# hmetaxa/MVTopicModel

Hardware: AMD Instinct MI355X
Metric: gibbs_tokens_per_sec (higher is better)
Workload: dtype f64

## Files before the change

### include/mvhdp.h

```cpp
#ifndef MVHDP_H
#define MVHDP_H

#include <stddef.h>
#include <stdint.h>

#ifdef __cplusplus
extern "C" {
#endif

#define MVHDP_MAX_MODALITIES 8
#define MVHDP_MAX_TOPICS     2048
#define MVHDP_UNASSIGNED_TOPIC (-1)

typedef enum {
    MVHDP_OK = 0,
    MVHDP_ERR_INVALID_ARG   = -1,
    MVHDP_ERR_STATE         = -2,
    MVHDP_ERR_HIP           = -3,
    MVHDP_ERR_NO_DEVICE     = -4,
    MVHDP_ERR_NEGATIVE_COUNT= -5,
    MVHDP_ERR_UNSUPPORTED   = -6
} mvhdp_status;

typedef struct mvhdp_ctx* mvhdp_handle;
// ... 95 lines not shown
int mvhdp_build_counts(mvhdp_handle h);
int mvhdp_build_trees(mvhdp_handle h);
int mvhdp_build_inference_trees(mvhdp_handle h);
int mvhdp_init_assignments_from_trees(mvhdp_handle h, uint64_t seed);
int mvhdp_get_counts(mvhdp_handle h, int32_t m, int32_t* n_wk , int32_t* n_k );
int mvhdp_set_counts(mvhdp_handle h, int32_t m, const int32_t* n_wk, const int32_t* n_k);
int mvhdp_get_tree(mvhdp_handle h, int32_t m, int32_t type, double* tree );
int mvhdp_get_doc_topic_hist(mvhdp_handle h, int32_t m, int32_t* hist , int32_t hist_len,
                             int32_t* doc_len_counts , int32_t len_len);

int mvhdp_get_count_histogram(mvhdp_handle h, int32_t m, int32_t* hist, int32_t len);
int mvhdp_view_overlap_sums(mvhdp_handle h, double* sums );
int mvhdp_model_log_likelihood(mvhdp_handle h, double* log_likelihood );
int mvhdp_gamma_doc_statistics(mvhdp_handle h, int32_t m, double gamma_m, uint64_t seed, uint32_t round, double* qs, double* qw);
int mvhdp_dp_table_statistics(mvhdp_handle h, int32_t m, const int32_t* hist , int32_t hist_len, const double* conc ,
                              uint64_t seed, uint32_t round, double* mk , uint8_t* active );
int mvhdp_antoniak_draws(mvhdp_handle h, int32_t n, const int32_t* items , const double* conc , uint64_t seed, uint32_t round, int32_t* tables );
int mvhdp_doc_topic_proportions(mvhdp_handle h, const double* view_weights , int64_t d0, int64_t d1, double* out );

#define MVHDP_DIAG_MAX_TOP_WORDS 64
#define MVHDP_DIAG_PROPORTIONS   7
#define MVHDP_DIAG_TOKENS             0
#define MVHDP_DIAG_DOCUMENT_ENTROPY   1
#define MVHDP_DIAG_WORD_LENGTH        2
#define MVHDP_DIAG_COHERENCE          3
#define MVHDP_DIAG_NORM_DISCR_WEIGHT  4
#define MVHDP_DIAG_DISCR_WEIGHT       5
#define MVHDP_DIAG_UNIFORM_DIST       6
#define MVHDP_DIAG_CORPUS_DIST        7
#define MVHDP_DIAG_EFF_NUM_WORDS      8
#define MVHDP_DIAG_TOKEN_DOC_DIFF     9
#define MVHDP_DIAG_RANK_1_DOCS       10
#define MVHDP_DIAG_ALLOCATION_RATIO  11
#define MVHDP_DIAG_ALLOCATION_COUNT  12
#define MVHDP_DIAG_ROWS              13
typedef struct {
    int32_t num_top_words;
    const int32_t* word_length;
} mvhdp_diag_args;
typedef struct {
    double*  scores;
    double*  word_scores;
    int32_t* codoc;
    int32_t* top_types;
    int32_t* top_counts;
    int32_t* nonzero;
    int32_t* num_rank1_docs;
    int32_t* num_nonzero_docs;
    int32_t* num_docs_at_proportions;
    double*  sum_count_log_count;
    int32_t* word_type_counts;
    int64_t* num_tokens;
    double*  discr_weight_per_view;
} mvhdp_diag_out;
int mvhdp_top_words(mvhdp_handle h, int32_t m, int32_t n, int32_t* types , int32_t* counts , int32_t* nonzero );
int mvhdp_discr_weights(mvhdp_handle h, double* per_view , int32_t m, double* type_weight );
int mvhdp_diagnostics(mvhdp_handle h, const mvhdp_diag_args* args, mvhdp_diag_out* out);

int mvhdp_sweep(mvhdp_handle h, uint32_t sweep_idx, uint64_t seed, uint32_t flags,
                const double* p_override, const mvhdp_debug* dbg, mvhdp_sweep_stats* stats);
int mvhdp_sweep_many(mvhdp_handle h, uint32_t first_idx, int32_t n, uint64_t seed, uint32_t flags, mvhdp_sweep_stats* stats );
int mvhdp_apply_delta(mvhdp_handle h, int32_t activated_topic, int32_t activated_modality);
int mvhdp_apply_delta_begin(mvhdp_handle h);
int mvhdp_apply_delta_rows(mvhdp_handle h, int64_t row_begin, int64_t row_end);
int mvhdp_apply_delta_end(mvhdp_handle h, int32_t activated_topic, int32_t activated_modality);
int mvhdp_get_birth_keys(mvhdp_handle h, int64_t* keys );
int mvhdp_activate_births(mvhdp_handle h, const int64_t* keys );
int mvhdp_trees_current(mvhdp_handle h);
int mvhdp_get_view_weights(mvhdp_handle h, double* p );

typedef struct {
    int32_t force_primary;
    int32_t narrow;
    int32_t walk_fixed;
    int32_t single_stream;
    int32_t live16;
    int32_t single_wave;
    double  walk_theta[MVHDP_MAX_MODALITIES];
    double  primary_min_share;
    int32_t learnt_walk_step[4];
    double  tree_branch_share[MVHDP_MAX_MODALITIES];
    int32_t live_overlap;
    int32_t live_rows;
} mvhdp_tuning;
int mvhdp_get_tuning(mvhdp_handle h, mvhdp_tuning* t);
int mvhdp_set_tuning(mvhdp_handle h, const mvhdp_tuning* t);

typedef struct {
    int32_t num_topics, num_modalities;
    int64_t num_entities;
    int64_t max_entity_tokens;
    int64_t entities_longer_than[5];
    uint64_t tokens_by_list_rounds[17];
    uint64_t entities_by_class[8];
    uint32_t flags;
    int32_t debug, batch, trees_current;
    int32_t num_cus;
    int32_t kernel_registers[6][3];
    int32_t inactive_topics;
} mvhdp_plan_input;
typedef struct {
    int32_t status;
    int32_t segments, primary_class, register_resident, need_full_trees, dominant_class;
    int64_t routed_prefix;
    int32_t class_used[6], class_map[6], class_stream[6], class_grid[6], class_walk[6], class_narrow[6], class_register_resident[6];
    int64_t class_lds_bytes[6];
    double  class_theta0[6];
    int32_t delta16, live_rows;
} mvhdp_plan_output;
int mvhdp_plan_probe(const mvhdp_plan_input* in, const mvhdp_tuning* tuning , mvhdp_plan_output* out);
int mvhdp_tuner_probe(int32_t num_modalities, const double* tree_branch_share , const double* u1_hist ,
                      const double* ns_by_step , int32_t n_sweeps, int32_t group, int32_t* steps_out );

typedef struct mvhdp_group_ctx* mvhdp_group;
#define MVHDP_UNIQUE_ID_BYTES 128
typedef struct {
    int32_t local_members;
    int32_t local_devices;
    int32_t ranks, first_rank;
    int32_t rccl;
    int32_t rccl_version;
    int32_t exchange_chunks;
    int32_t exchange_packed;
    double  last_exchange_ms;
    int64_t last_exchange_bytes;
} mvhdp_group_info;
int mvhdp_group_create(int32_t n, const mvhdp_handle* members, mvhdp_group* out);
int mvhdp_group_unique_id(uint8_t* id );
int mvhdp_group_create_rank(mvhdp_handle member, const uint8_t* id , int32_t rank, int32_t nranks, mvhdp_group* out);
int mvhdp_group_destroy(mvhdp_group g);
const char* mvhdp_group_last_error(mvhdp_group g);
int mvhdp_group_get_info(mvhdp_group g, mvhdp_group_info* info);
int mvhdp_group_set_exchange_chunks(mvhdp_group g, int32_t chunks );
int mvhdp_group_build_counts(mvhdp_group g);
int mvhdp_group_sweep(mvhdp_group g, uint32_t sweep_idx, uint64_t seed, uint32_t flags, mvhdp_sweep_stats* stats);
#define MVHDP_SWEEP_ASYNC_EXCHANGE 0x100u
int mvhdp_group_drain(mvhdp_group g);
int mvhdp_group_abort(mvhdp_group g);

int mvhdp_group_set_hyper(mvhdp_group g, const mvhdp_hyper* hy);
int mvhdp_group_log_likelihood(mvhdp_group g, double* log_likelihood );
int mvhdp_group_doc_topic_hist(mvhdp_group g, int32_t m, int32_t* hist , int32_t hist_len,
                               int32_t* doc_len_counts , int32_t len_len);
int mvhdp_group_count_histogram(mvhdp_group g, int32_t m, int32_t* hist, int32_t len);
int mvhdp_group_view_overlap_sums(mvhdp_group g, double* sums );
int mvhdp_group_gamma_doc_statistics(mvhdp_group g, int32_t m, double gamma_m, uint64_t seed, uint32_t round, double* qs, double* qw);
int mvhdp_group_diagnostics(mvhdp_group g, const mvhdp_diag_args* args, mvhdp_diag_out* out);

int mvhdp_device_buffer(mvhdp_handle h, mvhdp_buffer which, void** dev_ptr, size_t* bytes);
int mvhdp_counts_written(mvhdp_handle h);
int mvhdp_set_stream(mvhdp_handle h, void* hip_stream );
int mvhdp_synchronize(mvhdp_handle h);

#ifdef __cplusplus
}
#endif
#endif
```

### mvtopicmodel_amd/_lib.py

```python
import ctypes as C
import os

_HERE = os.path.dirname(os.path.abspath(__file__))
LIB_PATH = os.path.join(_HERE, "lib", "libmvhdp.so")

MAX_M = 8

ABI_SYMBOLS = [
    "mvhdp_create", "mvhdp_destroy", "mvhdp_last_error", "mvhdp_version",
    "mvhdp_set_corpus", "mvhdp_set_assignments", "mvhdp_set_view_presence", "mvhdp_get_assignments",
    "mvhdp_set_hyper", "mvhdp_get_alpha", "mvhdp_build_counts", "mvhdp_build_trees",
    "mvhdp_build_inference_trees", "mvhdp_init_assignments_from_trees",
    "mvhdp_get_counts", "mvhdp_set_counts", "mvhdp_get_tree", "mvhdp_get_doc_topic_hist",
    "mvhdp_get_count_histogram", "mvhdp_view_overlap_sums", "mvhdp_model_log_likelihood", "mvhdp_doc_topic_proportions",
    "mvhdp_gamma_doc_statistics", "mvhdp_dp_table_statistics", "mvhdp_antoniak_draws",
    "mvhdp_top_words", "mvhdp_discr_weights", "mvhdp_diagnostics",
    "mvhdp_sweep", "mvhdp_sweep_many", "mvhdp_get_tuning", "mvhdp_set_tuning", "mvhdp_plan_probe", "mvhdp_tuner_probe",
    "mvhdp_apply_delta", "mvhdp_apply_delta_begin", "mvhdp_apply_delta_rows", "mvhdp_apply_delta_end",
    "mvhdp_get_birth_keys", "mvhdp_activate_births",
    "mvhdp_trees_current", "mvhdp_get_view_weights",
    "mvhdp_device_buffer", "mvhdp_counts_written", "mvhdp_set_stream", "mvhdp_synchronize",
    "mvhdp_group_create", "mvhdp_group_unique_id", "mvhdp_group_create_rank", "mvhdp_group_destroy", "mvhdp_group_last_error",
    "mvhdp_group_get_info", "mvhdp_group_set_exchange_chunks", "mvhdp_group_build_counts", "mvhdp_group_sweep", "mvhdp_group_abort", "mvhdp_group_drain",
    "mvhdp_group_set_hyper", "mvhdp_group_log_likelihood", "mvhdp_group_doc_topic_hist", "mvhdp_group_count_histogram",
    "mvhdp_group_view_overlap_sums", "mvhdp_group_gamma_doc_statistics", "mvhdp_group_diagnostics",
]

UNIQUE_ID_BYTES = 128


class MvhdpError(RuntimeError):
    def __init__(self, code, msg):
        super().__init__(f"mvhdp error {code}: {msg}")
        self.code = code


class Config(C.Structure):
    _fields_ = [("num_topics", C.c_int32), ("num_modalities", C.c_int32),
                ("num_types", C.c_int32 * MAX_M), ("device", C.c_int32),
                ("doc_id_base", C.c_int64), ("flags", C.c_uint32)]


class HyperC(C.Structure):
    _fields_ = [("alpha", C.c_void_p),
                ("alpha_sum", C.c_double * MAX_M), ("beta", C.c_double * MAX_M),
                ("beta_sum", C.c_double * MAX_M), ("gamma", C.c_double * MAX_M),
                ("p_a", (C.c_double * MAX_M) * MAX_M), ("p_b", (C.c_double * MAX_M) * MAX_M),
                ("inactive", C.c_void_p)]


class SweepStatsC(C.Structure):
    _fields_ = [("tokens", C.c_int64), ("changed", C.c_int64), ("new_mass_cnt", C.c_int64),
                ("topic_doc_mass_cnt", C.c_int64), ("word_ftree_mass_cnt", C.c_int64),
                ("oov_skipped", C.c_int64), ("aborted_docs", C.c_int64), ("exact_fallbacks", C.c_int64),
                ("activated_topic", C.c_int32), ("activated_modality", C.c_int32),
                ("activation_key", C.c_int64), ("sweep_kernel_ms", C.c_double), ("total_ms", C.c_double),
                ("activations", C.c_int32), ("reserved", C.c_int32)]


class DebugC(C.Structure):
    _fields_ = [("tok_dbg", C.c_void_p * MAX_M), ("n_trace", C.c_int32),
                ("trace_doc", C.c_void_p), ("trace_view", C.c_void_p), ("trace_pos", C.c_void_p),
                ("trace_out", C.c_void_p)]


class TuningC(C.Structure):
    _fields_ = [("force_primary", C.c_int32), ("narrow", C.c_int32), ("walk_fixed", C.c_int32), ("single_stream", C.c_int32),
                ("live16", C.c_int32), ("single_wave", C.c_int32),
                ("walk_theta", C.c_double * MAX_M), ("primary_min_share", C.c_double),
                ("learnt_walk_step", C.c_int32 * 4), ("tree_branch_share", C.c_double * MAX_M),
                ("live_overlap", C.c_int32), ("live_rows", C.c_int32)]


class GroupInfoC(C.Structure):
    _fields_ = [("local_members", C.c_int32), ("local_devices", C.c_int32), ("ranks", C.c_int32), ("first_rank", C.c_int32),
                ("rccl", C.c_int32), ("rccl_version", C.c_int32), ("exchange_chunks", C.c_int32), ("exchange_packed", C.c_int32),
                ("last_exchange_ms", C.c_double), ("last_exchange_bytes", C.c_int64)]


class PlanInputC(C.Structure):
    _fields_ = [("num_topics", C.c_int32), ("num_modalities", C.c_int32), ("num_entities", C.c_int64),
                ("max_entity_tokens", C.c_int64), ("entities_longer_than", C.c_int64 * 5),
                ("tokens_by_list_rounds", C.c_uint64 * 17), ("entities_by_class", C.c_uint64 * 8),
                ("flags", C.c_uint32), ("debug", C.c_int32), ("batch", C.c_int32), ("trees_current", C.c_int32),
                ("num_cus", C.c_int32), ("kernel_registers", (C.c_int32 * 3) * 6), ("inactive_topics", C.c_int32)]


class PlanOutputC(C.Structure):
    _fields_ = [("status", C.c_int32), ("segments", C.c_int32), ("primary_class", C.c_int32), ("register_resident", C.c_int32),
                ("need_full_trees", C.c_int32), ("dominant_class", C.c_int32), ("routed_prefix", C.c_int64),
                ("class_used", C.c_int32 * 6), ("class_map", C.c_int32 * 6), ("class_stream", C.c_int32 * 6),
                ("class_grid", C.c_int32 * 6), ("class_walk", C.c_int32 * 6), ("class_narrow", C.c_int32 * 6),
                ("class_register_resident", C.c_int32 * 6), ("class_lds_bytes", C.c_int64 * 6), ("class_theta0", C.c_double * 6),
                ("delta16", C.c_int32), ("live_rows", C.c_int32)]


DIAG_MAX_TOP_WORDS = 64
DIAG_PROPORTIONS = 7
DIAG_ROWS = ["tokens", "document_entropy", "word-length", "coherence", "normDiscrWeight", "discrWeight", "uniform_dist",
             "corpus_dist", "eff_num_words", "token-doc-diff", "rank_1_docs", "allocation_ratio", "allocation_count"]


class DiagArgsC(C.Structure):
    _fields_ = [("num_top_words", C.c_int32), ("word_length", C.c_void_p)]


class DiagOutC(C.Structure):
    _fields_ = [("scores", C.c_void_p), ("word_scores", C.c_void_p), ("codoc", C.c_void_p), ("top_types", C.c_void_p),
                ("top_counts", C.c_void_p), ("nonzero", C.c_void_p), ("num_rank1_docs", C.c_void_p), ("num_nonzero_docs", C.c_void_p),
                ("num_docs_at_proportions", C.c_void_p), ("sum_count_log_count", C.c_void_p), ("word_type_counts", C.c_void_p),
                ("num_tokens", C.c_void_p), ("discr_weight_per_view", C.c_void_p)]


_lib = None
_preloaded = []


def _torch_lib_dir():
    import importlib.util
    try:
        spec = importlib.util.find_spec("torch")
    except (ImportError, ValueError):
        return None
    if spec is None or not spec.submodule_search_locations:
        return None
    d = os.path.join(list(spec.submodule_search_locations)[0], "lib")
    return d if os.path.isdir(d) else None


def mapped_runtime_libraries():
    found = {"libamdhip64": set(), "libhsa-runtime64": set(), "librccl": set()}
    try:
        with open("/proc/self/maps") as f:
            for line in f:
                path = line.rsplit(None, 1)[-1] if "/" in line else ""
                base = os.path.basename(path)
                for name in found:
                    if base.startswith(name + ".so"):
                        found[name].add(os.path.realpath(path))
    except OSError:
        pass
    return {k: sorted(v) for k, v in found.items()}


def _preload_one_hip_runtime():
    d = _torch_lib_dir()
    if d is None:
        return False
    already = mapped_runtime_libraries()
    if already["libamdhip64"] or already["libhsa-runtime64"]:
        return False
    path = os.path.join(d, "libamdhip64.so")
    if not os.path.exists(path):
        return False
# ... 96 lines not shown
```

### mvtopicmodel_amd/csrc/mvhdp_api.hip

```cpp
#include "mvhdp_ctx.h"

static thread_local std::string g_create_error;

static std::mutex g_reg_mutex;
static std::set<mvhdp_ctx*>* g_live = nullptr;
static bool g_exiting = false, g_atexit_registered = false;
static void release_device_resources(mvhdp_ctx* h);

static void mvhdp_at_exit()
{
    std::lock_guard<std::mutex> lk(g_reg_mutex);
    g_exiting = true;
    if (g_live) for (mvhdp_ctx* h : *g_live) release_device_resources(h);
}

static void register_handle(mvhdp_ctx* h)
{
    std::lock_guard<std::mutex> lk(g_reg_mutex);
    if (!g_live) g_live = new std::set<mvhdp_ctx*>();
    g_live->insert(h);
    if (!g_atexit_registered) { atexit(mvhdp_at_exit); g_atexit_registered = true; }
}

bool mvhdp_is_live(mvhdp_ctx* h)
{
    std::lock_guard<std::mutex> lk(g_reg_mutex);
    return g_live && g_live->count(h) != 0;
}

static void read_environment(mvhdp_ctx* h)
{
    if (const char* f = getenv("MVHDP_FORCE_RMAX")) { const int v = atoi(f); if (v == 1 || v == 2 || v == 4 || v == 8 || v == 16 || v == 32) h->tu.force_primary = v; }
    if (const char* f = getenv("MVHDP_NARROW")) h->tu.narrow = atoi(f) != 0 ? -1 : 0;
    if (const char* f = getenv("MVHDP_SINGLE_STREAM")) h->tu.single_stream = atoi(f) != 0;
    if (const char* f = getenv("MVHDP_SIDE_PRIORITY")) h->side_priority = atoi(f);
    if (const char* f = getenv("MVHDP_LIVE16")) h->tu.live16 = atoi(f);
    if (const char* f = getenv("MVHDP_LIVE_OVERLAP")) h->tu.live_overlap = atoi(f);
    if (const char* f = getenv("MVHDP_LIVE_ROWS")) h->tu.live_rows = atoi(f);
    if (const char* f = getenv("MVHDP_LIVE_ROWS_THETA")) h->tu.live_rows_theta = atof(f);
    if (const char* f = getenv("MVHDP_COEF_LDS_KB")) h->tu.coef_lds_max_bytes = std::max(0, std::min(64, atoi(f))) * 1024;
    if (const char* f = getenv("MVHDP_LIVE_ROWS_SEGMENTS")) h->tu.live_rows_segments = std::max(1, std::min(255, atoi(f)));
    if (const char* f = getenv("MVHDP_WIDEST_ON_MAIN")) h->tu.widest_on_main = atoi(f) != 0;
    if (const char* f = getenv("MVHDP_NARROW_WIDE")) h->tu.narrow_wide = atoi(f) != 0;
    if (const char* f = getenv("MVHDP_LIVE_TREE_EVERY")) h->live_tree_every = std::max(1, atoi(f));
    if (const char* f = getenv("MVHDP_GATE_PCT")) { const int v = atoi(f); if (v >= 5 && v <= 95) h->gate_pct = v; }
    if (const char* f = getenv("MVHDP_FOUR_ROUND_ON_C")) h->tu.four_round_on_c = atoi(f);
    if (const char* f = getenv("MVHDP_DELTA16")) h->tu.delta16 = atoi(f) != 0;
    if (const char* f = getenv("MVHDP_FORK_DELAY_US")) h->tu.fork_delay_us = std::max(0, std::min(1000, atoi(f)));
    if (const char* f = getenv("MVHDP_FORCE_MODE")) { if (!strcmp(f, "serial")) h->tu.single_stream = 1; }
    if (const char* f = getenv("MVHDP_PRIMARY_MIN_SHARE")) { const double v = atof(f); if (v > 0.0 && v <= 1.0) h->tu.primary_min_share = v; }
    if (const char* t = getenv("MVHDP_WALK_THETA")) {
        int m = 0;
        for (const char* q = t; *q && m < MVHDP_MAXM; m++) {
            h->tu.walk_theta[m] = atof(q);
            while (*q && *q != ',') q++;
            if (*q == ',') q++;
        }
        for (; m < MVHDP_MAXM; m++) h->tu.walk_theta[m] = 0.0;
        h->tu.walk_fixed = 1;
    }
    h->dbg_env = getenv("MVHDP_DEBUG") != nullptr;
}

extern "C" const char* mvhdp_version(void) { return "mvhdp 0.1 (gfx950)"; }

extern "C" const char* mvhdp_last_error(mvhdp_handle h) { return (h && mvhdp_is_live(h)) ? h->err.c_str() : g_create_error.c_str(); }

extern "C" int mvhdp_create(const mvhdp_config* cfg, mvhdp_handle* out)
{
    if (!cfg || !out) { g_create_error = "null argument"; return MVHDP_ERR_INVALID_ARG; }
    *out = nullptr;
    const int K = cfg->num_topics, M = cfg->num_modalities;
    if (K < 1 || K > MVHDP_MAX_TOPICS || M < 1 || M > MVHDP_MAX_MODALITIES) {
        g_create_error = "num_topics must be in [1,2048] and num_modalities in [1,8]";
        return MVHDP_ERR_INVALID_ARG;
    }
    for (int m = 0; m < M; m++) if (cfg->num_types[m] < 1) { g_create_error = "num_types[m] must be >= 1"; return MVHDP_ERR_INVALID_ARG; }
    for (int m = 0; m < M; m++) if (cfg->num_types[m] >= (1 << 29)) { g_create_error = "num_types[m] must be below 2^29"; return MVHDP_ERR_INVALID_ARG; }
    if (cfg->doc_id_base < 0 || cfg->doc_id_base >= (1LL << 29)) { g_create_error = "doc_id_base out of range"; return MVHDP_ERR_INVALID_ARG; }
    int ndev = 0;
    if (hipGetDeviceCount(&ndev) != hipSuccess || ndev <= 0 || cfg->device < 0 || cfg->device >= ndev) {
        g_create_error = "no usable HIP device (the sweep has no CPU fallback)";
        return MVHDP_ERR_NO_DEVICE;
    }
    hipDeviceProp_t prop;
    if (hipGetDeviceProperties(&prop, cfg->device) != hipSuccess) { g_create_error = "hipGetDeviceProperties failed"; return MVHDP_ERR_HIP; }
    if (strncmp(prop.gcnArchName, "gfx950", 6) != 0) {
        g_create_error = std::string("device is ") + prop.gcnArchName + ", this library is built for gfx950 only";
        return MVHDP_ERR_NO_DEVICE;
    }
    mvhdp_ctx* h = new mvhdp_ctx();
    register_handle(h);
    h->cfg = *cfg;
    h->device = cfg->device;
    h->num_cus = prop.multiProcessorCount;
    h->max_lds = 160 * 1024;
    MvModel& mm = h->mm;
    mm.K = K; mm.M = M;
    mm.rowbase[0] = 0;
    for (int m = 0; m < M; m++) { mm.V[m] = cfg->num_types[m]; mm.rowbase[m + 1] = mm.rowbase[m] + cfg->num_types[m]; }
    mm.doc_id_base = cfg->doc_id_base;
    mm.first_inactive = -1;
    mm.D = -1;
#define CREATE_HIP(call) do { hipError_t e_ = (call); if (e_ != hipSuccess) { \
    g_create_error = std::string(#call) + ": " + hipGetErrorString(e_); mvhdp_destroy(h); return MVHDP_ERR_HIP; } } while (0)
    CREATE_HIP(hipSetDevice(h->device));
    CREATE_HIP(hipStreamCreateWithFlags(&h->stream, hipStreamNonBlocking));
    h->own_stream = true;
    for (auto& e : h->ev) CREATE_HIP(hipEventCreate(&e));
    const int64_t nrows = mm.rowbase[M];
    const size_t cbytes = (size_t)(nrows * K + (int64_t)M * K + MVHDP_TAIL_WORDS) * sizeof(int32_t);
    CREATE_HIP(hipMalloc(&mm.counts, cbytes));
    CREATE_HIP(hipMalloc(&mm.delta, cbytes));
    CREATE_HIP(hipMemset(mm.counts, 0, cbytes));
    CREATE_HIP(hipMalloc(&mm.counts16, (size_t)nrows * K * sizeof(uint16_t) + 64));
    CREATE_HIP(hipMemset(mm.counts16, 0, (size_t)nrows * K * sizeof(uint16_t)));
    CREATE_HIP(hipMalloc(&mm.delta16, (size_t)(nrows * K + 2) * sizeof(uint16_t)));
    CREATE_HIP(hipMemsetD16(mm.delta16, (unsigned short)0x8000, (size_t)(nrows * K + 2)));
    CREATE_HIP(hipMalloc(&mm.heavy, (size_t)nrows));
    CREATE_HIP(hipMemset(mm.heavy, 1, (size_t)nrows));
    CREATE_HIP(hipMemset(mm.delta, 0, cbytes));
    CREATE_HIP(hipMalloc(&mm.trees, (size_t)nrows * 2 * K * sizeof(double)));
    CREATE_HIP(hipMalloc(&mm.root, (size_t)nrows * sizeof(double)));
    CREATE_HIP(hipMalloc(&mm.mass0, (size_t)nrows * sizeof(float)));
    CREATE_HIP(hipMemset(mm.mass0, 0, (size_t)nrows * sizeof(float)));
    CREATE_HIP(hipMalloc(&mm.coef, (size_t)M * (((K + 7) & ~7) + K + 8) * sizeof(float)));
    {
        const int nlev = (K > 1) ? (32 - __builtin_clz((unsigned)(K - 1))) : 0;
        mm.dt_f = nlev ? ((nlev - 1) % 3) + 1 : 0;
        mm.dt_nbd = 1; mm.dt_base[0] = 0; mm.dt_depth[0] = 0;
        int nblk = 1;
        for (int dep = mm.dt_f; nlev && dep < nlev; dep += 3) {
            mm.dt_base[mm.dt_nbd] = nblk; mm.dt_depth[mm.dt_nbd] = dep; mm.dt_nbd++;
            nblk += 1 << dep;
        }
        mm.dt_nblk = nblk;
        CREATE_HIP(hipMalloc(&mm.dtab, (size_t)nrows * nblk * 8 * sizeof(double)));
    }
    CREATE_HIP(hipMalloc(&h->d_alpha, (size_t)M * (K + 1) * sizeof(double)));
    CREATE_HIP(hipMalloc(&h->d_inactive, (size_t)K));
    CREATE_HIP(hipMemset(h->d_inactive, 0, (size_t)K));
    CREATE_HIP(hipMalloc(&h->d_births, (size_t)(2 + 2 * K) * sizeof(int32_t)));
    CREATE_HIP(hipMemset(h->d_births, 0, (size_t)(2 + 2 * K) * sizeof(int32_t)));
    CREATE_HIP(hipMalloc(&h->d_birth_keys, (size_t)K * sizeof(long long)));
    CREATE_HIP(hipMalloc(&h->d_birth_table, (size_t)K * sizeof(long long)));
    {
        const std::vector<long long> none((size_t)K, LLONG_MAX);
        CREATE_HIP(hipMemcpy(h->d_birth_table, none.data(), (size_t)K * sizeof(long long), hipMemcpyHostToDevice));
    }
    CREATE_HIP(hipMalloc(&h->d_ctl, CTL_WORDS * sizeof(unsigned long long)));
    CREATE_HIP(hipMemset(h->d_ctl, 0, CTL_WORDS * sizeof(unsigned long long)));
    h->d_stats = h->d_ctl;
    h->d_act_key = (long long*)(h->d_ctl + ST_COUNT);
    h->d_ovf_meta = (unsigned int*)(h->d_ctl + ST_COUNT + 1);
    h->d_doc_counter = h->d_ctl + ST_COUNT + 1 + META_WORDS64;
    CREATE_HIP(hipHostMalloc((void**)&h->h_ctl, CTL_WORDS * sizeof(unsigned long long), hipHostMallocDefault));
    for (int c = 0; c < MVHDP_N_CLASSES; c++)
        for (int f = 0; f < 3; f++) h->regs.regs[c][f] = mvhdp_sweep_kernel_regs(c, f);
    read_environment(h);
    mm.alpha = h->d_alpha;
    mm.inactive = h->d_inactive;
    h->h_alpha.assign((size_t)M * (K + 1), 0.0);
    h->h_inactive.assign((size_t)K, 0);
    h->wt.init_defaults(K);
    *out = h;
    return MVHDP_OK;
}

static void release_device_resources(mvhdp_ctx* h)
{
    if (h->device_released) return;
    h->device_released = true;
    hipSetDevice(h->device);
    if (h->stream) hipStreamSynchronize(h->stream);
    auto fr = [](auto*& p) { if (p) { hipFree((void*)p); p = nullptr; } };
    for (int m = 0; m < MVHDP_MAXM; m++) { fr(h->d_doc_off[m]); fr(h->d_tok[m]); fr(h->d_z[m]); fr(h->d_carry[m]); fr(h->d_present[m]); }
    fr(h->mm.counts); fr(h->mm.delta16); fr(h->mm.counts16); fr(h->mm.heavy); fr(h->mm.delta); fr(h->mm.trees); fr(h->mm.root); fr(h->mm.coef); fr(h->mm.mass0); fr(h->d_births); fr(h->d_birth_keys); fr(h->d_birth_table); fr(h->mm.dtab); fr(h->mm.p);
    fr(h->d_alpha); fr(h->d_inactive); fr(h->d_ctl);
    if (h->h_ctl) { hipHostFree(h->h_ctl); h->h_ctl = nullptr; }
    h->d_stats = nullptr; h->d_act_key = nullptr; h->d_doc_counter = nullptr; h->d_ovf_meta = nullptr;
    fr(h->d_doc_order); fr(h->d_lists); fr(h->d_nslots); fr(h->d_stats_many); fr(h->d_heavy_list); fr(h->d_heavy_ctl);
    if (h->ev_rf_go) { hipEventDestroy(h->ev_rf_go); h->ev_rf_go = nullptr; }
    if (h->ev_rf_done) { hipEventDestroy(h->ev_rf_done); h->ev_rf_done = nullptr; }
    if (h->rf_stream) { hipStreamDestroy(h->rf_stream); h->rf_stream = nullptr; }
    fr(h->ov.counts2); fr(h->ov.counts16_2); fr(h->ov.dtab2); fr(h->ov.root2); fr(h->ov.trees2); fr(h->ov.delta2); fr(h->ov.delta3); fr(h->ov.ctl2); fr(h->ov.lists2);
    for (auto& e : h->ov.ev_seg) if (e) { hipEventDestroy(e); e = nullptr; }
    if (h->ov.ev_start) { hipEventDestroy(h->ov.ev_start); h->ov.ev_start = nullptr; }
    if (h->ov.x1) { hipStreamDestroy(h->ov.x1); h->ov.x1 = nullptr; }
    if (h->ov.xa) { hipStreamDestroy(h->ov.xa); h->ov.xa = nullptr; }
    for (auto& e : h->ev_many) if (e) { hipEventDestroy(e); e = nullptr; }
    for (auto& e : h->ev) if (e) { hipEventDestroy(e); e = nullptr; }
    if (h->ev_fork) { hipEventDestroy(h->ev_fork); h->ev_fork = nullptr; }
    for (auto& e : h->ev_join) if (e) { hipEventDestroy(e); e = nullptr; }
    for (auto& st : h->side) if (st) { hipStreamDestroy(st); st = nullptr; }
    if (h->own_stream && h->stream) hipStreamDestroy(h->stream);
    h->stream = nullptr;
}

extern "C" int mvhdp_destroy(mvhdp_handle h)
{
    if (!h) return MVHDP_OK;
    bool exiting;
    {
        std::lock_guard<std::mutex> lk(g_reg_mutex);
        if (!g_live || g_live->erase(h) == 0) return MVHDP_ERR_INVALID_ARG;
        exiting = g_exiting;
    }
    if (!exiting) release_device_resources(h);
    delete h;
    return MVHDP_OK;
}

extern "C" int mvhdp_set_stream(mvhdp_handle h, void* hip_stream)
{
    CHECK_H(h);
    HIPC(h, hipSetDevice(h->device));
    HIPC(h, hipStreamSynchronize(h->stream));
    if (h->own_stream) { hipStreamDestroy(h->stream); h->own_stream = false; }
    if (hip_stream) h->stream = (hipStream_t)hip_stream;
    else { HIPC(h, hipStreamCreateWithFlags(&h->stream, hipStreamNonBlocking)); h->own_stream = true; }
    return MVHDP_OK;
}

extern "C" int mvhdp_synchronize(mvhdp_handle h)
{
    CHECK_H(h);
    HIPC(h, hipSetDevice(h->device));
    HIPC(h, hipStreamSynchronize(h->stream));
    return MVHDP_OK;
}

extern "C" int mvhdp_set_corpus(mvhdp_handle h, int32_t m, int64_t D, const int64_t* doc_off, const int32_t* tokens)
{
    CHECK_H(h);
    MvModel& mm = h->mm;
    if (m < 0 || m >= mm.M || D < 0 || !doc_off) FAIL(h, MVHDP_ERR_INVALID_ARG, "set_corpus: bad view, num_docs or doc_off");
    if (mm.D >= 0 && D != mm.D) {
        bool any_other = false;
        for (int j = 0; j < mm.M; j++) if (j != m && h->have_corpus[j]) any_other = true;
        if (any_other) FAIL(h, MVHDP_ERR_INVALID_ARG, "set_corpus: every view must list the same entities (empty span = view absent)");
    }
    if (mm.doc_id_base + D >= (1LL << 29)) FAIL(h, MVHDP_ERR_INVALID_ARG, "set_corpus: too many entities");
    if (doc_off[0] != 0) FAIL(h, MVHDP_ERR_INVALID_ARG, "set_corpus: doc_off[0] must be 0");
    for (int64_t d = 0; d < D; d++) {
        int64_t len = doc_off[d + 1] - doc_off[d];
        if (len < 0) FAIL(h, MVHDP_ERR_INVALID_ARG, "set_corpus: doc_off must be non-decreasing");
        if (len >= (1 << 20)) FAIL(h, MVHDP_ERR_INVALID_ARG, "set_corpus: a view of one entity is limited to 2^20-1 tokens");
    }
    const int64_t N = doc_off[D];
    if (N > 0 && !tokens) FAIL(h, MVHDP_ERR_INVALID_ARG, "set_corpus: tokens is null");
    HIPC(h, hipSetDevice(h->device));
    HIPC(h, hipStreamSynchronize(h->stream));
    if (h->d_doc_off[m]) { hipFree(h->d_doc_off[m]); h->d_doc_off[m] = nullptr; }
    if (h->d_tok[m]) { hipFree(h->d_tok[m]); h->d_tok[m] = nullptr; }
    if (h->d_z[m]) { hipFree(h->d_z[m]); h->d_z[m] = nullptr; }
    if (h->d_present[m]) { hipFree(h->d_present[m]); h->d_present[m] = nullptr; }
    h->h_present[m].clear(); mm.present[m] = nullptr;
    HIPC(h, hipMalloc(&h->d_doc_off[m], (size_t)(D + 1) * sizeof(int64_t)));
    HIPC(h, hipMemcpy(h->d_doc_off[m], doc_off, (size_t)(D + 1) * sizeof(int64_t), hipMemcpyHostToDevice));
    const size_t nb = (size_t)std::max<int64_t>(N, 1) * sizeof(int32_t);
// ... 746 lines not shown
        MvModel mk;
        if (p.seg_apply) {
            mk = B[seg == 0 ? 0 : (seg - 1) & 1];
            mk.delta = D3[seg % 3];
        } else {
            mk = mm;
            mk.delta = mm.counts;
            mk.dtab = B[seg & 1].dtab; mk.root = B[seg & 1].root; mk.trees = B[seg & 1].trees;
            if (seg >= 1 && !(flags & MVHDP_SWEEP_REUSE_TREES)) {
                step(hipStreamWaitEvent(xs, ev_reset(seg - 1), 0));
                const int64_t n_prev = share_of(seg - 1, mm.D), H_prev = p.route ? share_of(seg - 1, p.H) : 0;
                const unsigned long long thr = (unsigned long long)((n_prev - H_prev) * h->gate_pct / 100);
                step(mvhdp_launch_gate(ctl[(seg - 1) & 1].qheads + p.pc, thr, xs));
                MvModel tm = mm;
                tm.dtab = mk.dtab; tm.root = mk.root; tm.trees = mk.trees;
                if (p.live16) step(mvhdp_launch_build_trees_from_mirror(tm, p.need_full, xs, true));
                else step(mvhdp_launch_build_trees(tm, false, p.need_full, xs, true));
            } else if (seg >= 1) {
                mk.dtab = mm.dtab; mk.root = mm.root; mk.trees = mm.trees;
            }
        }
        step(mvhdp_launch_ctl_reset(nullptr, 0, nullptr, nullptr, 0, cs.class_counts, cs.qheads, xs));
        step(hipEventRecord(ev_reset(seg), xs));
        step(launch_segment_kernels(h, p, mk, sl, seg, xs, cs, d_stats));
        step(hipEventRecord(ev_done(seg), xs));
        if (p.seg_apply) {
            if (seg >= 1) step(hipStreamWaitEvent(xs, ev_applied(seg - 1), 0));
            const MvModel& dst = B[(seg + 1) & 1];
            step(mvhdp_launch_apply2_counts(dst, D3[seg % 3], seg >= 1 ? D3[(seg - 1) % 3] : nullptr, use_mirror, d_stats + ST_NEGATIVE, xs));
            step(hipEventRecord(ev_applied(seg), xs));
        }
    }
    if (mm.D > 0 && e == hipSuccess) {
        if (p.seg_apply) {
            step(hipStreamWaitEvent(X[0], ev_applied(nseg - 1), 0));
            if (nseg >= 2) step(hipStreamWaitEvent(X[0], ev_done(nseg - 2), 0));
            const MvModel& last = B[(nseg + 1) & 1];
            step(mvhdp_launch_apply_sparse(last, D3[(nseg - 1) % 3], use_mirror, X[0]));
            h->have_trees = false;
        } else {
            step(hipStreamWaitEvent(X[0], ev_done(nseg - 1), 0));
            if (nseg >= 2) step(hipStreamWaitEvent(X[0], ev_done(nseg - 2), 0));
        }
    }
    if (p.live) {
        if (p.live16 && mm.D > 0) { step(mvhdp_launch_widen_mirror(mm, X[0])); h->have_trees = false; }
        if (flags & MVHDP_SWEEP_NO_APPLY) {
            step(mvhdp_launch_live_helper(mm, 1, d_stats, X[0]));
            if (!(flags & MVHDP_SWEEP_REUSE_TREES)) h->have_trees = false;
        } else step(mvhdp_launch_live_helper(mm, 2, d_stats, X[0]));
        if (!(flags & MVHDP_SWEEP_REUSE_TREES)) h->have_trees = false;
    }
    step(hipEventRecord(ev_k1, X[0]));
    if (e != hipSuccess) HIPC(h, e);
    return MVHDP_OK;
}

static int enqueue_sweep(mvhdp_ctx* h, const SweepPlan& p, uint32_t sweep_idx, uint64_t seed, const double* p_override,
                         const DebugBufs* db, unsigned long long* d_stats, hipEvent_t ev_k0, hipEvent_t ev_k1, SweepOutcome& oc)
{
    if (p.overlap) return enqueue_overlapped(h, p, sweep_idx, seed, p_override, d_stats, ev_k0, ev_k1);
    MvModel& mm = h->mm;
    const int M = mm.M;
    const uint32_t flags = p.flags;
    const int nseg = p.nseg;
    hipStream_t s = h->stream;
    hipError_t e = hipSuccess;
    auto step = [&](hipError_t r) { if (e == hipSuccess) e = r; };

    SweepLaunch sl{};
    sl.sweep_idx = sweep_idx; sl.seed_lo = (uint32_t)seed; sl.seed_hi = (uint32_t)(seed >> 32);
    sl.flags = flags & 0x7fffu; sl.S_cap = p.S_cap;
    if (h->tu.single_wave && p.live) sl.flags |= MVHDP_SL_STRICT_LIVE;
    if (p.live_rows && getenv("MVHDP_NO_ROW_SAMPLE")) sl.flags |= 0x2000u;
#ifdef MVHDP_PROBE
    if (const char* f = getenv("MVHDP_ATOMIC_PROBE")) sl.flags |= ((unsigned)atoi(f) & 7u) << 16;
#endif
    sl.q_order_stride = 1;
    sl.nk_global = p.nk_global; sl.block_shared_bytes = p.block_shared_bytes;
    sl.live16 = p.live16 ? 1 : 0;
    sl.live_rows = p.live_rows ? 1 : 0;
    sl.coef_lds = p.coef_lds ? 1 : 0;
    sl.delta16 = p.delta16 ? 1 : 0;
    sl.stats = d_stats;
    sl.act_key = h->d_act_key;
    const bool births = sweep_births(p, flags, mm);
    if (births) { sl.births = h->d_births; sl.birth_keys = h->d_birth_keys; }
    sl.slot_hist = (unsigned long long*)h->d_ovf_meta + META_HIST;
    if (db) {
        for (int m = 0; m < M; m++) sl.tok_dbg[m] = db->tok_dbg[m];
        sl.n_trace = db->n_trace; sl.trace_doc = db->trace_doc; sl.trace_view = db->trace_view; sl.trace_pos = db->trace_pos; sl.trace_out = db->trace_out;
    }
    unsigned int* class_counts = h->d_ovf_meta + META_CLASS_COUNTS;

    if (M > 1) {
        if (!mm.p && mm.D > 0) step(hipMalloc(&mm.p, (size_t)mm.D * M * M * sizeof(double)));
        if (e == hipSuccess) {
            if (p_override) step(hipMemcpyAsync(mm.p, p_override, (size_t)mm.D * M * M * sizeof(double), hipMemcpyHostToDevice, s));
            else step(mvhdp_launch_draw_p(mm, sweep_idx, sl.seed_lo, sl.seed_hi, s));
        }
    }
    h->last_need_full = p.need_full;
    const bool dummy_poll = getenv("MVHDP_DUMMY_POLL") != nullptr;
    const bool refresher = ((p.live_rows && p.live16) || dummy_poll) && !h->tu.single_wave && !getenv("MVHDP_NO_HEAVY_REFRESH");
    auto live_rows_prepare = [&](bool from_mirror) -> hipError_t {
        if ((p.live16 || dummy_poll) && !h->d_heavy_list) {
            hipError_t e1 = hipMalloc(&h->d_heavy_list, (size_t)MVHDP_HEAVY_CAP * sizeof(int32_t));
            if (e1 == hipSuccess) e1 = hipMalloc(&h->d_heavy_ctl, 2 * sizeof(unsigned int));
            if (e1 != hipSuccess) return e1;
        }
        if (refresher && !h->rf_stream) {
            int least = 0, greatest = 0;
            if (hipDeviceGetStreamPriorityRange(&least, &greatest) != hipSuccess || greatest >= least ||
                hipStreamCreateWithPriority(&h->rf_stream, hipStreamNonBlocking, greatest) != hipSuccess) {
                (void)hipGetLastError(); h->rf_stream = nullptr;
                hipError_t e1 = hipStreamCreateWithFlags(&h->rf_stream, hipStreamNonBlocking); if (e1 != hipSuccess) return e1;
            }
            hipError_t e1 = hipEventCreateWithFlags(&h->ev_rf_go, hipEventDisableTiming);
            if (e1 == hipSuccess) e1 = hipEventCreateWithFlags(&h->ev_rf_done, hipEventDisableTiming);
            if (e1 != hipSuccess) return e1;
        }
        return mvhdp_launch_live_rows_prepare(mm, from_mirror, p.live16, p.live16 ? h->d_heavy_list : nullptr, p.live16 ? h->d_heavy_ctl : nullptr, MVHDP_HEAVY_CAP,
                                              p.live16 ? 512 : 256 , s);
    };
    auto rebuild_trees = [&]() {
        step(mvhdp_launch_build_trees(mm, false, p.need_full, s));
        h->have_trees = true; h->full_trees = p.need_full; h->trees_inference = false;
    };
    if (p.live_rows) {
        step(live_rows_prepare(false));
        h->have_trees = false; h->full_trees = false;
    } else if (!(flags & MVHDP_SWEEP_REUSE_TREES)) rebuild_trees();
    if (dummy_poll && !p.live_rows) {
        if (!h->d_heavy_list) { step(hipMalloc(&h->d_heavy_list, (size_t)MVHDP_HEAVY_CAP * sizeof(int32_t))); step(hipMalloc(&h->d_heavy_ctl, 2 * sizeof(unsigned int))); }
        if (!h->rf_stream) { step(hipStreamCreateWithFlags(&h->rf_stream, hipStreamNonBlocking)); step(hipEventCreateWithFlags(&h->ev_rf_go, hipEventDisableTiming)); step(hipEventCreateWithFlags(&h->ev_rf_done, hipEventDisableTiming)); }
        step(hipMemsetAsync(h->d_heavy_ctl, 0, 2 * sizeof(unsigned int), s));
    }
    else if (p.need_full && !h->full_trees) {
        step(mvhdp_launch_build_trees(mm, h->trees_inference, true, s));
        h->full_trees = true;
    }
    MvModel mk = mm;
    if (p.live) {
        mk.delta = mm.counts;
        if (flags & MVHDP_SWEEP_NO_APPLY) { step(mvhdp_launch_live_helper(mm, 0, d_stats, s)); h->delta_clean = false; }
    } else if (!p.frozen) {
        if (!h->delta_clean) {
            step(hipMemsetAsync(mm.delta, 0, (size_t)counts_len(h) * sizeof(int32_t), s));
            if (h->delta16_used) step(hipMemsetD16Async(mm.delta16, (unsigned short)0x8000, (size_t)(mm.rowbase[M] * mm.K), s));
            h->delta16_used = false;
        }
        h->delta_clean = false;
        if (p.delta16) h->delta16_used = true;
    }
    step(mvhdp_launch_ctl_reset(d_stats, ST_COUNT, h->d_act_key, (unsigned long long*)h->d_ovf_meta, META_WORDS64, nullptr, h->d_doc_counter, s));
    if (births) step(births_begin(h, s));
    step(hipEventRecord(ev_k0, s));

    const int seg_lo = p.only_seg >= 0 ? p.only_seg : 0, seg_hi = p.only_seg >= 0 ? p.only_seg + 1 : nseg;
    for (int seg = seg_lo; seg < seg_hi && e == hipSuccess && mm.D > 0; seg++) {
        if (seg > seg_lo) {
            if (births && !(flags & MVHDP_SWEEP_NO_APPLY) && e == hipSuccess) {
                const int rc = births_end(h, s, oc);
                if (rc != MVHDP_OK) return rc;
                mk.first_inactive = mm.first_inactive;
                step(births_begin(h, s));
// ... 260 lines not shown
{
    CHECK_H(h);
    if (n < 0) FAIL(h, MVHDP_ERR_INVALID_ARG, "sweep_many: n < 0");
    if (n == 0) return MVHDP_OK;
    MvModel& mm = h->mm;
    const bool frozen = (flags & MVHDP_SWEEP_FROZEN) != 0;
    if (n == 1 || mm.first_inactive >= 0 || ((flags & MVHDP_SWEEP_NO_APPLY) && !frozen) || ((flags & MVHDP_SWEEP_REUSE_TREES) && !frozen) || n > 4096) {
        for (int i = 0; i < n; i++) {
            const int rc = mvhdp_sweep(h, first_idx + (uint32_t)i, seed, flags, nullptr, nullptr, stats ? stats + i : nullptr);
            if (rc) return rc;
        }
        return MVHDP_OK;
    }
    int rc = sweep_preconditions(h, flags); if (rc) return rc;
    HIPC(h, hipSetDevice(h->device));
    hipStream_t s = h->stream;
    rc = ensure_slot_counts(h); if (rc) return rc;
    PlanIn in; fill_plan_in(h, flags, false, true, in);
    SweepPlan p;
    plan_sweep(in, h->tu, h->wt, p);
    if (p.err) FAIL(h, p.err, p.msg);
    rc = set_generic_lds(h, p); if (rc) return rc;
    if (h->dbg_env) debug_print_plan(h, p, first_idx);
    if (h->stats_many_cap < n) {
        if (h->d_stats_many) { hipFree(h->d_stats_many); h->d_stats_many = nullptr; h->stats_many_cap = 0; }
        HIPC(h, hipMalloc(&h->d_stats_many, (size_t)n * ST_COUNT * sizeof(unsigned long long)));
        h->stats_many_cap = n;
    }
    while ((int)h->ev_many.size() < 2 * n) { hipEvent_t ev; HIPC(h, hipEventCreate(&ev)); h->ev_many.push_back(ev); }
    HIPC(h, hipEventRecord(h->ev[0], s));
    for (int i = 0; i < n; i++) {
        SweepOutcome oc;
        unsigned long long* d_st = h->d_stats_many + (size_t)i * ST_COUNT;
        rc = enqueue_sweep(h, p, first_idx + (uint32_t)i, seed, nullptr, nullptr, d_st, h->ev_many[2 * i], h->ev_many[2 * i + 1], oc);
        if (rc) return rc;
        if (!p.frozen && !p.live && !p.seg_apply) {
            HIPC(h, mvhdp_launch_apply_delta(mm, d_st, s, h->delta16_used));
            h->delta16_used = false;
            h->have_trees = false; h->delta_clean = true;
        } else if (p.live || p.seg_apply) {
            h->have_trees = false;
            if (p.seg_apply) h->delta_clean = true;
        }
    }
    HIPC(h, hipEventRecord(h->ev[3], s));
    std::vector<unsigned long long> hs((size_t)n * ST_COUNT);
    unsigned long long meta[META_WORDS64] = {0};
    HIPC(h, hipMemcpyAsync(hs.data(), h->d_stats_many, hs.size() * sizeof(unsigned long long), hipMemcpyDeviceToHost, s));
    HIPC(h, hipMemcpyAsync(meta, h->d_ovf_meta, sizeof meta, hipMemcpyDeviceToHost, s));
    HIPC(h, hipStreamSynchronize(s));
    if (p.seg_apply && p.overlap) h->ov.deltas_dirty = false;
    float ms_t = 0;
    hipEventElapsedTime(&ms_t, h->ev[0], h->ev[3]);
    int ret = MVHDP_OK;
    double ms_sum = 0;
    for (int i = 0; i < n; i++) {
        const unsigned long long* hi = hs.data() + (size_t)i * ST_COUNT;
        mvhdp_sweep_stats st;
        stats_from_counters(hi, LLONG_MAX, st);
        float ms_k = 0;
        hipEventElapsedTime(&ms_k, h->ev_many[2 * i], h->ev_many[2 * i + 1]);
        st.sweep_kernel_ms = ms_k; st.total_ms = ms_t / n;
        ms_sum += ms_k;
        if (stats) stats[i] = st;
        if (hi[ST_MISCLASS]) { h->nslots_valid = false; FAIL(h, MVHDP_ERR_HIP, "internal: an entity reached a sweep kernel variant that cannot hold its topic list"); }
        if (hi[ST_NEGATIVE] && ret == MVHDP_OK) { h->err = "a topic count went below zero (UPD:202-215)"; ret = MVHDP_ERR_NEGATIVE_COUNT; }
    }
    if (meta[META_MISROUTED]) { h->nslots_valid = false; FAIL(h, MVHDP_ERR_HIP, "internal: an entity could not be routed to a sweep kernel"); }
    std::vector<unsigned long long> acc(ST_COUNT, 0);
    for (int i = 0; i < n; i++) for (int k = 0; k < ST_COUNT; k++) acc[k] += hs[(size_t)i * ST_COUNT + k];
    const bool comparable = p.fast && !h->tu.walk_fixed && !(flags & (MVHDP_SWEEP_FROZEN | MVHDP_SWEEP_EXACT_CHAIN));
    learn_from_sweep(h, p, acc.data(), meta + META_HIST, ms_sum, comparable);
    if (!p.frozen && acc[ST_ABORT] == 0) for (int m = 0; m < mm.M; m++) h->unassigned[m] = false;
    return ret;
}

extern "C" int mvhdp_get_tuning(mvhdp_handle h, mvhdp_tuning* t)
{
    CHECK_H(h);
    if (!t) FAIL(h, MVHDP_ERR_INVALID_ARG, "get_tuning: null");
    memset(t, 0, sizeof *t);
    t->force_primary = h->tu.force_primary; t->narrow = h->tu.narrow; t->walk_fixed = h->tu.walk_fixed;
    t->single_stream = h->tu.single_stream; t->primary_min_share = h->tu.primary_min_share; t->live16 = h->tu.live16;
    t->single_wave = h->tu.single_wave; t->live_overlap = h->tu.live_overlap; t->live_rows = h->tu.live_rows;
    for (int m = 0; m < MVHDP_MAX_MODALITIES; m++) { t->walk_theta[m] = h->tu.walk_theta[m]; t->tree_branch_share[m] = h->wt.walk_f[m]; }
    for (int g = 0; g < WALK_GROUPS; g++) t->learnt_walk_step[g] = g == h->wt.walk_cls ? h->wt.walk_i : h->wt.walk_i_by[g];
    t->learnt_walk_step[3] = -1;
    return MVHDP_OK;
}

extern "C" int mvhdp_set_tuning(mvhdp_handle h, const mvhdp_tuning* t)
{
    CHECK_H(h);
    if (!t) FAIL(h, MVHDP_ERR_INVALID_ARG, "set_tuning: null");
    const int fp = t->force_primary;
    if (!(fp == 0 || fp == 1 || fp == 2 || fp == 4 || fp == 8 || fp == 16 || fp == 32)) FAIL(h, MVHDP_ERR_INVALID_ARG, "set_tuning: force_primary must be 0, 1, 2, 4, 8, 16 or 32");
    if (t->primary_min_share < 0.0 || t->primary_min_share > 1.0) FAIL(h, MVHDP_ERR_INVALID_ARG, "set_tuning: primary_min_share outside [0, 1]");
    for (int g = 0; g < WALK_GROUPS; g++) if (t->learnt_walk_step[g] < -1 || t->learnt_walk_step[g] > MVHDP_WALK_BINS) FAIL(h, MVHDP_ERR_INVALID_ARG, "set_tuning: learnt_walk_step outside [-1, 20]");
    h->tu.force_primary = fp; h->tu.narrow = t->narrow; h->tu.walk_fixed = t->walk_fixed ? 1 : 0;
    h->tu.single_stream = t->single_stream ? 1 : 0;
    h->tu.live16 = t->live16 < 0 ? -1 : (t->live16 ? 1 : 0);
    h->tu.single_wave = t->single_wave ? 1 : 0;
    h->tu.live_overlap = t->live_overlap < 0 ? -1 : (t->live_overlap ? 1 : 0);
    h->tu.live_rows = t->live_rows < 0 ? -1 : (t->live_rows ? 1 : 0);
    h->tu.primary_min_share = t->primary_min_share > 0.0 ? t->primary_min_share : 0.10;
    for (int m = 0; m < MVHDP_MAX_MODALITIES; m++) h->tu.walk_theta[m] = t->walk_theta[m];
    if (t->learnt_walk_step[0] >= 0 || t->learnt_walk_step[1] >= 0 || t->learnt_walk_step[2] >= 0) h->wt.restore(t->learnt_walk_step, t->tree_branch_share, h->mm.M);
    return MVHDP_OK;
}

extern "C" int mvhdp_plan_probe(const mvhdp_plan_input* pi, const mvhdp_tuning* t, mvhdp_plan_output* po)
{
    if (!pi || !po) return MVHDP_ERR_INVALID_ARG;
    PlanIn in;
    in.K = pi->num_topics; in.M = pi->num_modalities; in.D = pi->num_entities; in.mdt = pi->max_entity_tokens;
    if (in.K < 1 || in.K > MVHDP_MAX_TOPICS || in.M < 1 || in.M > MVHDP_MAX_MODALITIES || in.D < 0) return MVHDP_ERR_INVALID_ARG;
    in.have_order = true;
    for (int c = 0; c < 5; c++) in.n_longer[c] = pi->entities_longer_than[c];
    for (int b = 0; b < MVHDP_HIST_BINS; b++) in.tok_hist[b] = pi->tokens_by_list_rounds[b];
    for (int b = 0; b < MVHDP_ENT_BINS; b++) in.ent_hist[b] = pi->entities_by_class[b];
    in.flags = pi->flags; in.debug = pi->debug != 0; in.batch = pi->batch != 0; in.trees_current = pi->trees_current != 0;
    in.first_inactive = pi->inactive_topics ? 0 : -1;
    in.num_cus = pi->num_cus > 0 ? pi->num_cus : 256;
    for (int c = 0; c < MVHDP_N_CLASSES; c++) for (int f = 0; f < 3; f++) in.regs.regs[c][f] = pi->kernel_registers[c][f];
    PlanTuning tu;
    WalkTuner wt;
    wt.init_defaults(in.K);
    if (t) {
        tu.force_primary = t->force_primary; tu.narrow = t->narrow; tu.walk_fixed = t->walk_fixed; tu.single_stream = t->single_stream;
        tu.live16 = t->live16; tu.single_wave = t->single_wave ? 1 : 0; tu.live_overlap = t->live_overlap; tu.live_rows = t->live_rows;
        if (t->primary_min_share > 0) tu.primary_min_share = t->primary_min_share;
        for (int m = 0; m < MVHDP_MAX_MODALITIES; m++) tu.walk_theta[m] = t->walk_theta[m];
        if (t->learnt_walk_step[0] >= 0 || t->learnt_walk_step[1] >= 0 || t->learnt_walk_step[2] >= 0) wt.restore(t->learnt_walk_step, t->tree_branch_share, in.M);
    }
    SweepPlan p;
    plan_sweep(in, tu, wt, p);
    memset(po, 0, sizeof *po);
    po->status = p.err;
    if (p.err) return MVHDP_OK;
    po->segments = p.nseg; po->primary_class = p.pc; po->routed_prefix = p.H; po->register_resident = p.fast ? 1 : 0;
    po->need_full_trees = p.need_full ? 1 : 0; po->dominant_class = p.dominant;
    for (int c = 0; c < MVHDP_N_CLASSES; c++) {
        po->class_used[c] = p.cls[c].used ? 1 : 0; po->class_map[c] = p.class_map[c];
        po->class_stream[c] = p.cls[c].stream; po->class_grid[c] = p.cls[c].grid; po->class_lds_bytes[c] = (int64_t)p.cls[c].lds;
        po->class_walk[c] = p.cls[c].walk; po->class_narrow[c] = p.cls[c].narrow; po->class_register_resident[c] = p.cls[c].fast ? 1 : 0;
        po->class_theta0[c] = p.cls[c].theta[0];
    }
    po->delta16 = p.delta16 ? 1 : 0;
    po->live_rows = p.live_rows ? 1 : 0;
    return MVHDP_OK;
}

extern "C" int mvhdp_tuner_probe(int32_t num_modalities, const double* tree_branch_share, const double* u1_hist, const double* ns_by_step ,
                                 int32_t n_sweeps, int32_t group, int32_t* steps_out )
{
    if (!tree_branch_share || !ns_by_step || !steps_out || num_modalities < 1 || num_modalities > MVHDP_MAX_MODALITIES || n_sweeps < 0) return MVHDP_ERR_INVALID_ARG;
    WalkTuner wt;
    if (group < 0 || group >= WALK_GROUPS) return MVHDP_ERR_INVALID_ARG;
    for (int m = 0; m < num_modalities; m++) wt.walk_f[m] = tree_branch_share[m];
    for (int b = 0; b < MVHDP_WALK_BINS; b++) wt.walk_hist[b] = u1_hist ? u1_hist[b] : 0.0;
    for (int i = 0; i < n_sweeps; i++) {
        double theta[WALK_GROUPS][MVHDP_MAXM]; bool measure;
        wt.propose(group, num_modalities, theta, &measure);
        steps_out[i] = wt.walk_probe_i;
        wt.observe(true, 1, num_modalities, ns_by_step[std::max(0, std::min(MVHDP_WALK_BINS, wt.walk_probe_i))]);
    }
    return MVHDP_OK;
}

extern "C" int mvhdp_get_view_weights(mvhdp_handle h, double* p)
{
    CHECK_H(h);
    MvModel& mm = h->mm;
    if (!p) FAIL(h, MVHDP_ERR_INVALID_ARG, "get_view_weights: null");
    if (mm.M == 1) { for (int64_t d = 0; d < mm.D; d++) p[d] = 1.0; return MVHDP_OK; }
    if (!mm.p) FAIL(h, MVHDP_ERR_STATE, "get_view_weights before the first sweep");
    HIPC(h, hipSetDevice(h->device));
    HIPC(h, hipStreamSynchronize(h->stream));
    HIPC(h, hipMemcpy(p, mm.p, (size_t)mm.D * mm.M * mm.M * sizeof(double), hipMemcpyDeviceToHost));
    return MVHDP_OK;
}

extern "C" int mvhdp_device_buffer(mvhdp_handle h, mvhdp_buffer which, void** dev_ptr, size_t* bytes)
{
    CHECK_H(h);
    if (!dev_ptr || !bytes) FAIL(h, MVHDP_ERR_INVALID_ARG, "device_buffer: null");
    size_t b = (size_t)counts_len(h) * sizeof(int32_t);
    if (which == MVHDP_BUF_COUNTS) { *dev_ptr = h->mm.counts; *bytes = b; return MVHDP_OK; }
    if (which == MVHDP_BUF_DELTA) { *dev_ptr = h->mm.delta; *bytes = b; return MVHDP_OK; }
    if (which == MVHDP_BUF_BIRTH_KEYS) { *dev_ptr = h->d_birth_table; *bytes = (size_t)h->mm.K * sizeof(long long); return MVHDP_OK; }
    FAIL(h, MVHDP_ERR_INVALID_ARG, "device_buffer: unknown buffer");
}

extern "C" int mvhdp_counts_written(mvhdp_handle h)
{
    CHECK_H(h);
    h->have_counts = true; h->have_trees = false; h->counts_stale = false;
    return MVHDP_OK;
}

static double log_gamma_stirling_host(double z)
{
    const double HALF_LOG_TWO_PI = std::log(6.283185307179586) / 2.0;
    int shift = 0;
    while (z < 2.0) { z = z + 1; shift++; }
    double result = HALF_LOG_TWO_PI + (z - 0.5) * std::log(z) - z + 1 / (12.0 * z) - 1 / (360.0 * z * z * z)
                    + 1 / (1260.0 * z * z * z * z * z);
    while (shift > 0) { shift--; z = z - 1; result = result - std::log(z); }
    return result;
}

extern "C" int mvhdp_get_count_histogram(mvhdp_handle h, int32_t m, int32_t* hist, int32_t len)
{
// ... 237 lines not shown
```

### mvtopicmodel_amd/csrc/mvhdp_device.h

```cpp
#pragma once
#include <hip/hip_runtime.h>
#include <stdint.h>

#define MVHDP_MAXM 8
#define MVHDP_WALK_BINS 20
#define MVHDP_VIEW_STATS (2 + MVHDP_WALK_BINS)

struct MvModel {
    int32_t K, M;
    int32_t V[MVHDP_MAXM];
    int64_t rowbase[MVHDP_MAXM + 1];
    int64_t D;
    int64_t doc_id_base;
    const int64_t* doc_off[MVHDP_MAXM];
    const int32_t* tok[MVHDP_MAXM];
    int32_t* z[MVHDP_MAXM];
    const uint8_t* present[MVHDP_MAXM];
    uint16_t* nslots;
    int32_t* counts;
    uint16_t* delta16;
    uint16_t* counts16;
    uint8_t* heavy;
    int32_t* delta;
    double* trees;
    double* root;
    float* coef;
    float* mass0;
    double* dtab;
    int32_t dt_nblk, dt_nbd, dt_f;
    int32_t dt_base[6], dt_depth[6];
    const double* alpha;
    const uint8_t* inactive;
    double alpha_sum[MVHDP_MAXM], beta[MVHDP_MAXM], beta_sum[MVHDP_MAXM], gamma[MVHDP_MAXM];
    double p_a[MVHDP_MAXM][MVHDP_MAXM], p_b[MVHDP_MAXM][MVHDP_MAXM];
    double* p;
    int32_t first_inactive;
};

#define MVHDP_SL_STRICT_LIVE 0x8000u
#define MVHDP_ROW_HEAVY 1
#define MVHDP_ROW_BIG 2

struct SweepLaunch {
    uint32_t sweep_idx;
    uint32_t seed_lo, seed_hi;
    uint32_t flags;
    int32_t  S_cap;
    int32_t  waves_per_block;
    uint32_t block_shared_bytes;
    int32_t  nk_global;
    uint32_t wave_bytes;
    unsigned long long* stats;
    long long* act_key;
    int32_t* births;
    long long* birth_keys;
    unsigned long long* doc_counter;
    const int32_t* q_list;
    const unsigned int* q_list_count;
    const int32_t* q_order;
    int64_t q_order_start, q_order_count, q_order_stride;
    double walk_theta[MVHDP_MAXM];
    int32_t walk;
    int32_t narrow;
    int32_t delta16;
    int32_t live16;
    int32_t live_rows;
    int32_t coef_lds;
    unsigned long long* slot_hist;
    double* tok_dbg[MVHDP_MAXM];
    int32_t n_trace;
    const int64_t* trace_doc; const int32_t* trace_view; const int32_t* trace_pos;
    double* trace_out;
};

enum {
    ST_TOKENS = 0, ST_CHANGED, ST_NEW, ST_DOC, ST_TREE, ST_OOV, ST_ABORT, ST_FALLBACK, ST_NEGATIVE, ST_MISCLASS, ST_ONDEMAND,
    ST_VIEW_BASE, ST_VIEW_LAST = ST_VIEW_BASE + MVHDP_VIEW_STATS * MVHDP_MAXM - 1,
    ST_T_QUEUE, ST_T_PROLOGUE, ST_T_VIEW, ST_T_CHUNK_HEAD, ST_T_TOKENS, ST_T_CHUNK_END, ST_T_TOTAL,
    ST_T_ENT0, ST_T_ENT1, ST_T_ENT2, ST_N_ENT0, ST_N_ENT1, ST_N_ENT2, ST_T_INIT, ST_T_FLUSH, ST_N_WAVES, ST_T_ROWS, ST_T_ROWS_WAIT,
    ST_COUNT
};

size_t mvhdp_sweep_wave_bytes(int M, int S_cap);

hipError_t mvhdp_launch_build_counts(const MvModel& mm, const int64_t* n_tokens_per_view, hipStream_t s);
hipError_t mvhdp_launch_build_trees(const MvModel& mm, bool inference_leaves, bool write_full, hipStream_t s, bool beside_samplers = false);
hipError_t mvhdp_launch_build_trees_rows(const MvModel& mm, bool inference_leaves, bool write_full, int64_t row_begin, int64_t row_end,
                                         bool apply_first, unsigned long long* negatives, hipStream_t s);
hipError_t mvhdp_launch_build_trees_from_mirror(const MvModel& mm, bool write_full, hipStream_t s, bool beside_samplers = false);
hipError_t mvhdp_launch_widen_mirror(const MvModel& mm, hipStream_t s);
hipError_t mvhdp_launch_live_rows_prepare(const MvModel& mm, bool from_mirror, bool with_heavy_trees, int32_t* heavy_list, unsigned int* heavy_ctl, int heavy_cap, int batch_cells, hipStream_t s);
hipError_t mvhdp_launch_heavy_refresh(const MvModel& mm, const int32_t* heavy_list, const unsigned int* ctl, int heavy_cap, int blocks, hipStream_t s);
hipError_t mvhdp_launch_set_u32(unsigned int* p, unsigned int v, hipStream_t s);
hipError_t mvhdp_launch_apply_nk(const MvModel& mm, unsigned long long* negatives, hipStream_t s);
hipError_t mvhdp_launch_apply2_counts(const MvModel& dst, const int32_t* dA, int32_t* dB, bool use_mirror, unsigned long long* negatives, hipStream_t s);
hipError_t mvhdp_launch_apply_sparse(const MvModel& dst, int32_t* d, bool use_mirror, hipStream_t s);
hipError_t mvhdp_launch_gate(const unsigned long long* qhead, unsigned long long threshold, hipStream_t s);
hipError_t mvhdp_launch_init_from_trees(const MvModel& mm, uint32_t seed_lo, uint32_t seed_hi, hipStream_t s);
hipError_t mvhdp_launch_draw_p(const MvModel& mm, uint32_t sweep_idx, uint32_t seed_lo, uint32_t seed_hi, hipStream_t s);
hipError_t mvhdp_launch_sweep(const MvModel& mm, const SweepLaunch& sl, int grid_blocks, bool debug, hipStream_t s);
hipError_t mvhdp_launch_apply_delta(const MvModel& mm, unsigned long long* stats, hipStream_t s, bool with_delta16 = false);
hipError_t mvhdp_launch_delay(int microseconds, hipStream_t s);
hipError_t mvhdp_launch_ctl_reset(unsigned long long* stats, int n_stats, long long* act_key, unsigned long long* meta, int n_meta,
                                  unsigned int* class_counts, unsigned long long* qheads, hipStream_t s);
hipError_t mvhdp_launch_birth_table(const int32_t* births, const long long* birth_keys, const long long* act_key, int K, long long* keys, hipStream_t s);
hipError_t mvhdp_launch_live_helper(const MvModel& mm, int which, unsigned long long* stats, hipStream_t s);
hipError_t mvhdp_launch_doc_topic_hist(const MvModel& mm, int m, int32_t* hist, int32_t hist_len,
                                       int32_t* doc_len_counts, int32_t len_len, hipStream_t s);
hipError_t mvhdp_sweep_set_max_lds(size_t bytes);
hipError_t mvhdp_launch_count_hist(const MvModel& mm, int m, int32_t* hist, int32_t len, hipStream_t s);
hipError_t mvhdp_launch_view_overlap(const MvModel& mm, double* out, hipStream_t s);
hipError_t mvhdp_launch_loglik_doc(const MvModel& mm, int m, double* doc_out, hipStream_t s);
hipError_t mvhdp_launch_loglik_topic(const MvModel& mm, int m, double* partial, int n_partial, unsigned long long* nonzero, hipStream_t s);
hipError_t mvhdp_launch_gamma_doc_stats(const MvModel& mm, int m, double gamma_m, uint32_t seed_lo, uint32_t seed_hi, uint32_t round,
                                        double* partial, int n_blocks, hipStream_t s);
hipError_t mvhdp_launch_dp_tables(const int32_t* hist, int hist_len, int K, int m, const double* conc, uint32_t seed_lo, uint32_t seed_hi, uint32_t round,
                                  double* mk, uint8_t* active, hipStream_t s);
hipError_t mvhdp_launch_antoniak_draws(int n, const int32_t* items, const double* conc, uint32_t seed_lo, uint32_t seed_hi, uint32_t round, int32_t* tables, hipStream_t s);
hipError_t mvhdp_launch_slot_hist(const MvModel& mm, unsigned long long* hist, hipStream_t s);
struct DocTopicCarry { const int64_t* src[MVHDP_MAXM]; };
hipError_t mvhdp_launch_doc_topic_prop(const MvModel& mm, const DocTopicCarry& carry, const double* w_dev, int64_t d0, int64_t d1, double* out_dev, hipStream_t s);
#define MVHDP_N_CLASSES 6
struct ClassifyArgs {
    const int32_t* order;
    int64_t n, start, stride;
    int32_t class_map[MVHDP_N_CLASSES];
    int32_t check_views;
    int32_t* lists[MVHDP_N_CLASSES];
    unsigned int* counts;
    unsigned long long* misrouted;
};
hipError_t mvhdp_launch_classify(const MvModel& mm, const ClassifyArgs& ca, hipStream_t s);
size_t mvhdp_sweep_fast_wave_bytes(int M, int S_cap, int rmax);
hipError_t mvhdp_launch_sweep_fast(const MvModel& mm, const SweepLaunch& sl, int rmax, int grid_blocks, bool debug, hipStream_t s);
int mvhdp_sweep_fast_occupancy(int rmax, bool debug, bool walk, int block_threads, size_t lds_bytes);
int mvhdp_sweep_generic_occupancy(bool debug, int block_threads, size_t lds_bytes);
int mvhdp_sweep_kernel_regs(int cls, int flavour);
int mvhdp_sweep_generic_regs(bool debug);

#define MVHDP_DOC_BATCH 2
#define MVHDP_HIST_BINS 17
#define MVHDP_ENT_BINS 8
#define MVHDP_NSLOTS_UNKNOWN 0xFFFFu

__host__ __device__ __forceinline__ int mvhdp_class_of(int n, bool view_beyond_16_bits)
{
// ... 67 lines not shown
```

### mvtopicmodel_amd/csrc/mvhdp_group.hip

```cpp
#include "mvhdp_ctx.h"

#include <dlfcn.h>
#include <rccl/rccl.h>

#include <map>

namespace {

struct Rccl {
    void* lib = nullptr;
    std::string path, why;
    ncclResult_t (*GetVersion)(int*) = nullptr;
    ncclResult_t (*GetUniqueId)(ncclUniqueId*) = nullptr;
    ncclResult_t (*CommInitRank)(ncclComm_t*, int, ncclUniqueId, int) = nullptr;
    ncclResult_t (*CommInitAll)(ncclComm_t*, int, const int*) = nullptr;
    ncclResult_t (*CommDestroy)(ncclComm_t) = nullptr;
    ncclResult_t (*AllReduce)(const void*, void*, size_t, ncclDataType_t, ncclRedOp_t, ncclComm_t, hipStream_t) = nullptr;
    ncclResult_t (*GroupStart)() = nullptr;
    ncclResult_t (*GroupEnd)() = nullptr;
    const char* (*GetErrorString)(ncclResult_t) = nullptr;
};

std::mutex g_rccl_mutex;
Rccl g_rccl;
// ... 363 lines not shown
    info->exchange_packed = g->pack_on ? 1 : 0;
    return MVHDP_OK;
}

extern "C" int mvhdp_group_set_exchange_chunks(mvhdp_group g, int32_t chunks)
{
    CHECK_G(g);
    if (chunks < 1 || chunks > 64) GFAIL(g, MVHDP_ERR_INVALID_ARG, "group_set_exchange_chunks: 1..64");
    g->chunks = chunks;
    return MVHDP_OK;
}

struct XErr {
    mvhdp_group_ctx* g;
    int rc = MVHDP_OK;
    void hip(hipError_t e, const char* what) { if (e != hipSuccess && rc == MVHDP_OK) { rc = MVHDP_ERR_HIP; g->err = std::string(what) + ": " + hipGetErrorString(e); } }
    void nccl(ncclResult_t r, const char* what) { if (r != ncclSuccess && rc == MVHDP_OK) { rc = MVHDP_ERR_HIP; g->err = std::string(what) + ": " + (g_rccl.GetErrorString ? g_rccl.GetErrorString(r) : "RCCL error"); } }
};

static int reduce_local(mvhdp_group_ctx* g, bool counts)
{
    XErr x{g};
    const int n = (int)g->members.size();
    for (int i = 0; i < n; i++) {
        const int li = g->leader_of[i];
        if (li == i) continue;
        mvhdp_ctx *h = g->members[i], *L = g->members[li];
        x.hip(hipSetDevice(L->device), "hipSetDevice");
        x.hip(hipStreamWaitEvent(L->stream, g->ev_swept[i], 0), "hipStreamWaitEvent");
        x.hip(launch_add_into(counts ? L->mm.counts : L->mm.delta, counts ? h->mm.counts : h->mm.delta, counts_len_of(L), L->stream), "add_into_kernel");
    }
    return x.rc;
}

static int allreduce_range(mvhdp_group_ctx* g, bool counts, int64_t e0, int64_t e1)
{
    if (e1 <= e0 || g->comms.empty()) return MVHDP_OK;
    Rccl* r = &g_rccl;
    XErr x{g};
    if (g->comms.size() > 1) x.nccl(r->GroupStart(), "ncclGroupStart");
    for (size_t l = 0; l < g->leaders.size(); l++) {
        mvhdp_ctx* L = g->members[g->leaders[l]];
        x.hip(hipSetDevice(L->device), "hipSetDevice");
        int32_t* buf = (counts ? L->mm.counts : L->mm.delta) + e0;
        x.nccl(r->AllReduce(buf, buf, (size_t)(e1 - e0), ncclInt32, ncclSum, g->comms[l], L->stream), "ncclAllReduce");
    }
    if (g->comms.size() > 1) x.nccl(r->GroupEnd(), "ncclGroupEnd");
    return x.rc;
}

static int fan_out_range(mvhdp_group_ctx* g, bool counts, int64_t e0, int64_t e1)
{
    if (e1 <= e0 || g->members.size() == g->leaders.size()) return MVHDP_OK;
    XErr x{g};
    for (size_t l = 0; l < g->leaders.size(); l++) {
        mvhdp_ctx* L = g->members[g->leaders[l]];
        x.hip(hipSetDevice(L->device), "hipSetDevice");
        x.hip(hipEventRecord(g->ev_reduced[l], L->stream), "hipEventRecord");
        for (size_t i = 0; i < g->members.size(); i++) {
            if (g->leader_of[i] != g->leaders[l] || (int)i == g->leaders[l]) continue;
            mvhdp_ctx* h = g->members[i];
            x.hip(hipStreamWaitEvent(h->stream, g->ev_reduced[l], 0), "hipStreamWaitEvent");
            const int32_t* src = (counts ? L->mm.counts : L->mm.delta) + e0;
            int32_t* dst = (counts ? h->mm.counts : h->mm.delta) + e0;
            x.hip(hipMemcpyAsync(dst, src, (size_t)(e1 - e0) * sizeof(int32_t), hipMemcpyDeviceToDevice, h->stream), "hipMemcpyAsync");
            x.hip(hipEventRecord(g->ev_swept[i], h->stream), "hipEventRecord");
            x.hip(hipStreamWaitEvent(L->stream, g->ev_swept[i], 0), "hipStreamWaitEvent");
        }
    }
    return x.rc;
}

static int pack_prepare(mvhdp_group_ctx* g)
{
    if (g->pack_ready || !g->pack_allowed) return MVHDP_OK;
    for (mvhdp_ctx* h : g->members) for (int m = 0; m < h->mm.M; m++) if (h->unassigned[m]) return MVHDP_OK;
    mvhdp_ctx* L0 = g->members[g->leaders[0]];
    const int64_t rows = L0->mm.rowbase[L0->mm.M];
    const int K = L0->mm.K;
    if (rows <= 0) return MVHDP_OK;
    std::vector<uint8_t> cls((size_t)rows);
    GHIP(g, hipSetDevice(L0->device));
    GHIP(g, hipMemcpy(cls.data(), L0->mm.heavy, (size_t)rows, hipMemcpyDeviceToHost));
    g->woff.assign((size_t)rows + 1, 0);
    for (int64_t r = 0; r < rows; r++) g->woff[(size_t)r + 1] = g->woff[(size_t)r] + (cls[(size_t)r] == 0 ? (K + 1) / 2 : K);
    if (g->d_woff.empty()) { g->d_woff.assign(g->leaders.size(), nullptr); g->d_cls.assign(g->leaders.size(), nullptr); g->xpack.assign(g->leaders.size(), nullptr); }
    for (size_t l = 0; l < g->leaders.size(); l++) {
        mvhdp_ctx* L = g->members[g->leaders[l]];
        GHIP(g, hipSetDevice(L->device));
        if (!g->d_woff[l]) GHIP(g, hipMalloc(&g->d_woff[l], (size_t)(rows + 1) * sizeof(int64_t)));
        if (!g->d_cls[l]) GHIP(g, hipMalloc(&g->d_cls[l], (size_t)rows));
        if (!g->xpack[l]) GHIP(g, hipMalloc(&g->xpack[l], (size_t)rows * K * sizeof(int32_t)));
        GHIP(g, hipMemcpy(g->d_woff[l], g->woff.data(), (size_t)(rows + 1) * sizeof(int64_t), hipMemcpyHostToDevice));
        GHIP(g, hipMemcpy(g->d_cls[l], cls.data(), (size_t)rows, hipMemcpyHostToDevice));
    }
    g->pack_hash = (int32_t)(g->woff[(size_t)rows] % 4091) + 1;
    g->pack_ready = true;
    return MVHDP_OK;
}

static void pack_reset(mvhdp_group_ctx* g) { g->pack_on = false; g->pack_ready = false; g->pack_hash = 0; g->sweeps_since_counts = 0; }

static int allreduce_rows_packed(mvhdp_group_ctx* g, int64_t r0, int64_t r1)
{
    XErr x{g};
    Rccl* r = &g_rccl;
    const int64_t w0 = g->woff[(size_t)r0], w1 = g->woff[(size_t)r1];
    const int K = g->members[0]->mm.K;
    const int grid = (int)std::min<int64_t>((r1 - r0 + 3) / 4, 8192);
    for (size_t l = 0; l < g->leaders.size(); l++) {
        mvhdp_ctx* L = g->members[g->leaders[l]];
        x.hip(hipSetDevice(L->device), "hipSetDevice");
        hipLaunchKernelGGL(pack_rows_kernel, dim3(std::max(grid, 1)), dim3(256), 0, L->stream, L->mm.delta, g->d_cls[l], g->d_woff[l], g->xpack[l], r0, r1, K);
        x.hip(hipGetLastError(), "pack_rows_kernel");
    }
    if (!g->comms.empty() && w1 > w0) {
        if (g->comms.size() > 1) x.nccl(r->GroupStart(), "ncclGroupStart");
        for (size_t l = 0; l < g->leaders.size(); l++) {
            mvhdp_ctx* L = g->members[g->leaders[l]];
            x.hip(hipSetDevice(L->device), "hipSetDevice");
            x.nccl(r->AllReduce(g->xpack[l] + w0, g->xpack[l] + w0, (size_t)(w1 - w0), ncclInt32, ncclSum, g->comms[l], L->stream), "ncclAllReduce");
        }
        if (g->comms.size() > 1) x.nccl(r->GroupEnd(), "ncclGroupEnd");
    }
    for (size_t l = 0; l < g->leaders.size(); l++) {
        mvhdp_ctx* L = g->members[g->leaders[l]];
        x.hip(hipSetDevice(L->device), "hipSetDevice");
        hipLaunchKernelGGL(unpack_rows_kernel, dim3(std::max(grid, 1)), dim3(256), 0, L->stream, L->mm.delta, g->d_cls[l], g->d_woff[l], g->xpack[l], r0, r1, K);
        x.hip(hipGetLastError(), "unpack_rows_kernel");
    }
    g->last_exchange_bytes += (w1 - w0) * (long long)sizeof(int32_t);
    return x.rc;
}

extern "C" int mvhdp_group_build_counts(mvhdp_group g)
{
    CHECK_G(g);
    DeviceGuard dg;
    if (g->async_pending) {
        for (size_t l = 0; l < g->leaders.size(); l++) { hipSetDevice(g->members[g->leaders[l]]->device); hipStreamSynchronize(g->comm[l]); }
        g->async_pending = false;
    }
    const int n = (int)g->members.size();
    const int64_t len = counts_len_of(g->members[0]);
    int local_err = MVHDP_OK;
    auto note = [&](int rc, const std::string& what) { if (rc != MVHDP_OK && local_err == MVHDP_OK) { local_err = rc; g->err = what; } };
    XErr x{g};
    pack_reset(g);
    for (int i = 0; i < n; i++) {
        mvhdp_ctx* h = g->members[i];
        const int rc = mvhdp_build_counts(h);
        if (rc != MVHDP_OK) note(rc, "member " + std::to_string(i) + ": " + h->err);
        if (!h->delta_clean) { x.hip(hipSetDevice(h->device), "hipSetDevice"); x.hip(hipMemsetAsync(h->mm.delta, 0, (size_t)(len + MVHDP_TAIL_WORDS) * sizeof(int32_t), h->stream), "hipMemsetAsync"); h->delta_clean = true; h->delta_pending = false; }
    }
    if (local_err != MVHDP_OK)
        for (int i = 0; i < n; i++) { mvhdp_ctx* h = g->members[i]; x.hip(hipSetDevice(h->device), "hipSetDevice"); x.hip(hipMemsetAsync(h->mm.counts, 0, (size_t)len * sizeof(int32_t), h->stream), "hipMemsetAsync"); }
    for (int i = 0; i < n; i++) { x.hip(hipSetDevice(g->members[i]->device), "hipSetDevice"); x.hip(hipEventRecord(g->ev_swept[i], g->members[i]->stream), "hipEventRecord"); }
    note(reduce_local(g, true), g->err);
    note(x.rc, g->err);
    for (size_t l = 0; l < g->leaders.size(); l++) {
        mvhdp_ctx* L = g->members[g->leaders[l]];
        x.hip(hipSetDevice(L->device), "hipSetDevice");
        hipLaunchKernelGGL(set_word_kernel, dim3(1), dim3(1), 0, L->stream, L->mm.counts + len, local_err != MVHDP_OK ? 1 : 0);
    }
    note(allreduce_range(g, true, 0, len + 1), g->err);
    note(fan_out_range(g, true, 0, len + 1), g->err);
// ... 661 lines not shown
```

### mvtopicmodel_amd/csrc/mvhdp_kernels.hip

```cpp
#include "mvhdp_device.h"
#include "../../include/mvhdp.h"

#include "mvhdp_wave.h"
#include <algorithm>

__global__ __launch_bounds__(256) void build_counts_kernel(MvModel mm, int m, int64_t n_tokens)
{
    extern __shared__ int nk_local[];
    const int K = mm.K;
    for (int i = threadIdx.x; i < K; i += blockDim.x) nk_local[i] = 0;
    __syncthreads();
    int32_t* nwk = mm.counts;
    const int64_t stride = (int64_t)gridDim.x * blockDim.x;
    for (int64_t i = (int64_t)blockIdx.x * blockDim.x + threadIdx.x; i < n_tokens; i += stride) {
        int topic = mm.z[m][i];
        if (topic == MVHDP_UNASSIGNED_TOPIC) continue;
        int type = mm.tok[m][i];
        if (type < 0 || type >= mm.V[m] || topic < 0 || topic >= K) continue;
        atomicAdd(&nk_local[topic], 1);
        atomicAdd(&nwk[(mm.rowbase[m] + type) * K + topic], 1);
    }
    __syncthreads();
    int32_t* nk = mm.counts + mm.rowbase[mm.M] * K + (int64_t)m * K;
    for (int i = threadIdx.x; i < K; i += blockDim.x)
// ... 1 lines not shown
}

hipError_t mvhdp_launch_build_counts(const MvModel& mm, const int64_t* n_tokens, hipStream_t s)
{
    const int K = mm.K;
    size_t total = (size_t)(mm.rowbase[mm.M] * K + (int64_t)mm.M * K) * sizeof(int32_t);
    hipError_t e = hipMemsetAsync(mm.counts, 0, total, s);
    if (e != hipSuccess) return e;
    for (int m = 0; m < mm.M; m++) {
        if (n_tokens[m] <= 0) continue;
        int64_t blocks = (n_tokens[m] + 255) / 256;
        int grid = (int)(blocks < 2048 ? blocks : 2048);
        hipLaunchKernelGGL(build_counts_kernel, dim3(grid), dim3(256), (size_t)K * sizeof(int), s, mm, m, n_tokens[m]);
        e = hipGetLastError();
        if (e != hipSuccess) return e;
    }
    return hipSuccess;
}

template <bool COHERENT = false>
__device__ __forceinline__ void tree_from_leaves(const MvModel& mm, int64_t row, double* t, int lane, bool write_full)
{
    const int K = mm.K;
    if (lane == 0) t[0] = 0.0;
    __syncthreads();
    if (K > 1) {
        int dmax = 31 - __clz(K - 1);
        for (int d = dmax; d >= 0; d--) {
            int lo = 1 << d, hi = min(2 << d, K);
            for (int i = lo + lane; i < hi; i += WAVE) t[i] = t[2 * i] + t[2 * i + 1];
            __syncthreads();
        }
    }
    if (write_full) {
        double* out = mm.trees + row * 2 * K;
        for (int i = lane; i < 2 * K; i += WAVE) out[i] = t[i];
    }
    if (lane == 0) { if (COHERENT) __hip_atomic_store(&mm.root[row], t[1], __ATOMIC_RELAXED, __HIP_MEMORY_SCOPE_AGENT); else mm.root[row] = t[1]; }
    double* dt = mm.dtab + row * (int64_t)mm.dt_nblk * 8;
    double2* o = (double2*)dt;
    for (int u = lane; u < mm.dt_nblk * 4; u += WAVE) {
        const int x = u >> 2, j = u & 3;
        int base = 0, dep = 0;
        if (x >= 1) {
            base = 1; dep = mm.dt_f;
            while (x >= base + (1 << dep)) { base += 1 << dep; dep += 3; }
        }
        const int b = (1 << dep) + (x - base);
        double v2[2];
#pragma unroll
        for (int h = 0; h < 2; h++) {
            const int q = 2 * j + h;
            const int node = (q == 0) ? b : (q < 3) ? 2 * b + (q - 1) : 4 * b + (q - 3);
            v2[h] = (q == 7) ? ((x == 0) ? t[1] : 0.0) : ((node < K) ? t[2 * node] : 0.0);
        }
        if (COHERENT) {
            __hip_atomic_store(&dt[2 * u], v2[0], __ATOMIC_RELAXED, __HIP_MEMORY_SCOPE_AGENT);
            __hip_atomic_store(&dt[2 * u + 1], v2[1], __ATOMIC_RELAXED, __HIP_MEMORY_SCOPE_AGENT);
        } else o[u] = make_double2(v2[0], v2[1]);
    }
    __syncthreads();
}

template <int TB>
__global__ __launch_bounds__(64) void build_trees_kernel(MvModel mm, bool inference_leaves, bool write_full, int64_t row_begin, int64_t row_end,
                                                         bool apply_first, unsigned long long* negatives, bool from_mirror, bool only_heavy = false)
{
    extern __shared__ double t[];
    const int K = mm.K, lane = threadIdx.x;
    const int64_t nrows = mm.rowbase[mm.M];
    const int32_t* nk_all = mm.counts + nrows * K;
    int neg = 0;
    __builtin_amdgcn_s_setprio(3);
    for (int64_t row = row_begin + blockIdx.x; row < row_end; row += gridDim.x) {
        if (only_heavy && mm.heavy[row] != MVHDP_ROW_HEAVY) continue;
        int m = 0;
        while (m + 1 < mm.M && row >= mm.rowbase[m + 1]) m++;
        int32_t* cnt = mm.counts + row * K;
        int32_t* dl = mm.delta + row * K;
        const int32_t* nk = nk_all + (int64_t)m * K;
        const double* al = mm.alpha + (int64_t)m * (K + 1);
        const double beta = mm.beta[m], beta_sum = mm.beta_sum[m], gamma = mm.gamma[m];
        uint16_t* c16 = mm.counts16 + row * K;
        const bool light_src = from_mirror && mm.heavy[row] != MVHDP_ROW_HEAVY;
        bool hv = false;
        if (!from_mirror) {
            long long sum = 0;
            for (int k0 = 0; k0 < K; k0 += WAVE * TB) {
                int cv[TB], dv[TB];
#pragma unroll
                for (int u = 0; u < TB; u++) {
                    const int k = k0 + u * WAVE + lane;
                    cv[u] = (k < K) ? cnt[k] : 0;
                    dv[u] = (apply_first && k < K) ? dl[k] : 0;
                }
#pragma unroll
                for (int u = 0; u < TB; u++) {
                    const int k = k0 + u * WAVE + lane;
                    if (k < K) {
                        int c = cv[u];
                        if (apply_first) {
                            const int d = dv[u];
                            if (d) { c += d; cnt[k] = c; dl[k] = 0; neg += c < 0; }
                        }
                        sum += c < 0 ? 70000 : c;
                    }
                }
            }
#pragma unroll
            for (int sft = 32; sft >= 1; sft >>= 1) sum += __shfl_xor(sum, sft, WAVE);
            hv = sum > 65534;
            if (lane == 0) mm.heavy[row] = hv ? MVHDP_ROW_HEAVY : (sum > 32767 ? MVHDP_ROW_BIG : 0);
        }
        for (int k0 = 0; k0 < K; k0 += WAVE * TB) {
            int cv[TB], nkv[TB];
            double alv[TB];
            bool inact[TB];
#pragma unroll
            for (int u = 0; u < TB; u++) {
                const int k = k0 + u * WAVE + lane;
                const bool in = k < K;
                cv[u] = in ? (light_src ? (int)c16[k] : cnt[k]) : 0;
                nkv[u] = in ? nk[k] : 0;
                alv[u] = (in && !inference_leaves) ? al[k] : 0.0;
                inact[u] = in && !inference_leaves && mm.inactive[k];
            }
#pragma unroll
            for (int u = 0; u < TB; u++) {
                const int k = k0 + u * WAVE + lane;
                if (k < K) {
                    const int c = cv[u];
                    if (light_src) cnt[k] = c;
                    else if (!from_mirror) c16[k] = hv ? (uint16_t)65535 : (uint16_t)c;
                    double leaf;
                    if (inference_leaves) {
                        leaf = ((double)c + beta) / ((double)nkv[u] + beta_sum);
                    } else if (inact[u]) {
                        leaf = 0.0;
                    } else {
                        double p_wt = ((double)c + beta) / ((double)nkv[u] + beta_sum);
                        leaf = gamma * alv[u] * p_wt;
                    }
                    t[K + k] = leaf;
                }
            }
        }
        tree_from_leaves(mm, row, t, lane, write_full);
    }
    if (apply_first && negatives) {
#pragma unroll
        for (int sft = 32; sft >= 1; sft >>= 1) neg += __shfl_xor(neg, sft, WAVE);
        if (lane == 0 && neg) atomicAdd(negatives, (unsigned long long)neg);
    }
}

hipError_t mvhdp_launch_build_trees(const MvModel& mm, bool inference_leaves, bool write_full, hipStream_t s, bool beside_samplers)
{
    if (!beside_samplers) return mvhdp_launch_build_trees_rows(mm, inference_leaves, write_full, 0, mm.rowbase[mm.M], false, nullptr, s);
    const int64_t nrows = mm.rowbase[mm.M];
    if (nrows <= 0) return hipSuccess;
    int grid = (int)(nrows < 65536 ? nrows : 65536);
    hipLaunchKernelGGL(build_trees_kernel<1>, dim3(grid), dim3(64), (size_t)2 * mm.K * sizeof(double), s, mm, inference_leaves, write_full,
                       (int64_t)0, nrows, false, (unsigned long long*)nullptr, false);
    return hipGetLastError();
}

hipError_t mvhdp_launch_build_trees_rows(const MvModel& mm, bool inference_leaves, bool write_full, int64_t row_begin, int64_t row_end,
                                         bool apply_first, unsigned long long* negatives, hipStream_t s)
{
    int64_t nrows = row_end - row_begin;
    if (nrows <= 0) return hipSuccess;
    int grid = (int)(nrows < 65536 ? nrows : 65536);
    if (mm.K > 512)
        hipLaunchKernelGGL(build_trees_kernel<8>, dim3(grid), dim3(64), (size_t)2 * mm.K * sizeof(double), s, mm, inference_leaves, write_full,
                           row_begin, row_end, apply_first, negatives, false);
    else
        hipLaunchKernelGGL(build_trees_kernel<4>, dim3(grid), dim3(64), (size_t)2 * mm.K * sizeof(double), s, mm, inference_leaves, write_full,
                           row_begin, row_end, apply_first, negatives, false);
    return hipGetLastError();
}

hipError_t mvhdp_launch_build_trees_from_mirror(const MvModel& mm, bool write_full, hipStream_t s, bool beside_samplers)
{
    const int64_t nrows = mm.rowbase[mm.M];
    if (nrows <= 0) return hipSuccess;
    int grid = (int)(nrows < 65536 ? nrows : 65536);
    if (beside_samplers)
        hipLaunchKernelGGL(build_trees_kernel<1>, dim3(grid), dim3(64), (size_t)2 * mm.K * sizeof(double), s, mm, false, write_full,
                           (int64_t)0, nrows, false, (unsigned long long*)nullptr, true);
    else if (mm.K > 512)
        hipLaunchKernelGGL(build_trees_kernel<8>, dim3(grid), dim3(64), (size_t)2 * mm.K * sizeof(double), s, mm, false, write_full,
                           (int64_t)0, nrows, false, (unsigned long long*)nullptr, true);
    else
        hipLaunchKernelGGL(build_trees_kernel<4>, dim3(grid), dim3(64), (size_t)2 * mm.K * sizeof(double), s, mm, false, write_full,
                           (int64_t)0, nrows, false, (unsigned long long*)nullptr, true);
    return hipGetLastError();
}

__global__ __launch_bounds__(256) void apply2_nk_kernel(int32_t* nk_dst, const int32_t* __restrict__ dA, int32_t* __restrict__ dB, int n, unsigned long long* negatives)
{
    const int i = blockIdx.x * blockDim.x + threadIdx.x;
    if (i >= n) return;
    int d = dA[i];
    if (dB) { const int d2 = dB[i]; if (d2) { d += d2; dB[i] = 0; } }
    if (d) { const int c = nk_dst[i] + d; nk_dst[i] = c; if (c < 0 && negatives) atomicAdd(negatives, 1ull); }
}

__global__ __launch_bounds__(256) void apply2_counts_kernel(MvModel mm, const int32_t* __restrict__ dA, int32_t* __restrict__ dB, bool use_mirror,
                                                           int64_t n_cells, int64_t n_all, unsigned long long* negatives)
{
    const int64_t stride = (int64_t)gridDim.x * blockDim.x;
    unsigned int* m32 = (unsigned int*)mm.counts16;
    const int K = mm.K;
    int neg = 0;
    __builtin_amdgcn_s_setprio(3);
    for (int64_t i = (int64_t)blockIdx.x * blockDim.x + threadIdx.x; i < n_all; i += stride) {
        int d = dA[i];
        if (dB) { const int d2 = dB[i]; if (d2) { d += d2; dB[i] = 0; } }
        if (!d) continue;
        const int old = __hip_atomic_fetch_add(&mm.counts[i], d, __ATOMIC_RELAXED, __HIP_MEMORY_SCOPE_AGENT);
        neg += old + d < 0;
        if (use_mirror && i < n_cells && mm.heavy[i / K] != MVHDP_ROW_HEAVY) __hip_atomic_fetch_add(&m32[i >> 1], (unsigned int)d << ((i & 1) * 16), __ATOMIC_RELAXED, __HIP_MEMORY_SCOPE_AGENT);
    }
    if (neg && negatives) atomicAdd(negatives, (unsigned long long)neg);
}

hipError_t mvhdp_launch_apply2_counts(const MvModel& dst, const int32_t* dA, int32_t* dB, bool use_mirror, unsigned long long* negatives, hipStream_t s)
{
    const int64_t cells = dst.rowbase[dst.M] * dst.K, all = cells + (int64_t)dst.M * dst.K;
// ... 1056 lines not shown
```

### mvtopicmodel_amd/csrc/mvhdp_plan.h

```cpp
#pragma once
#include <stdint.h>
#include <stddef.h>
#include <algorithm>
#include <cmath>
#include <cstring>

#include "mvhdp_device.h"
#include "../../include/mvhdp.h"

enum { PLAN_STREAM_MAIN = 0, PLAN_STREAM_A = 1, PLAN_STREAM_B = 2, PLAN_STREAM_C = 3, PLAN_STREAM_D = 4, PLAN_N_STREAMS = 5 };

struct PlanRegs { int regs[MVHDP_N_CLASSES][3]; };

struct PlanIn {
    int K = 0, M = 0;
    int64_t D = 0;
    int64_t mdt = 0;
    int64_t n_longer[5] = {0, 0, 0, 0, 0};
    bool have_order = false;
    unsigned long long tok_hist[MVHDP_HIST_BINS] = {0};
    unsigned long long ent_hist[MVHDP_ENT_BINS] = {0};
    uint32_t flags = 0;
    bool debug = false;
    bool batch = false;
    bool trees_current = false;
    bool unassigned = false;
    int first_inactive = -1;
    int num_cus = 256;
    size_t max_lds = 160 * 1024;
    PlanRegs regs{};
};

struct ClassLaunch {
    bool used = false;
    bool fast = false;
    int r = 0;
    int S_cap = 0;
    uint32_t wave_bytes = 0;
    int wpb = 0;
    size_t lds = 0;
    int grid = 0;
    int stream = PLAN_STREAM_MAIN;
    int walk = 0, narrow = 0;
    double theta[MVHDP_MAXM] = {0};
};

struct SweepPlan {
    int err = 0;
    const char* msg = "";
    uint32_t flags = 0;
    bool live = false, seg_apply = false, frozen = false, debug = false;
    bool overlap = false;
    int nseg = 1;
    int only_seg = -1;
    int S_cap = 0;
    bool fast = false;
    int pc = 0;
    bool route = false;
    int64_t H = 0;
    ClassLaunch cls[MVHDP_N_CLASSES];
    int class_map[MVHDP_N_CLASSES] = {0, 1, 2, 3, 4, 5};
    bool need_full = false;
    int nk_global = 0;
    uint32_t block_shared_bytes = 0;
    bool delta16 = false;
    bool live16 = false;
    bool live_rows = false;
    bool coef_lds = false;
    int dominant = 0;
    int walk_cfg = 0;
};

static inline double plan_class_tokens(const unsigned long long* tok_hist, int c)
{
    double t = 0;
    for (int b = 0; b < MVHDP_HIST_BINS; b++) {
        const int rounds = b + 1;
        int cb = 0;
        while (cb < 5 && rounds > (1 << cb)) cb++;
        if (b == MVHDP_HIST_BINS - 1) cb = 5;
        if (cb == c) t += (double)tok_hist[b];
    }
    return t;
}

static inline int plan_blocks_per_cu(int regs, int threads, size_t lds)
{
    int r = (regs + 7) / 8 * 8;
    int waves_simd = r > 0 ? 512 / r : 8;
    waves_simd = std::max(1, std::min(8, waves_simd));
    const int wpb = threads / 64;
    int b = waves_simd * 4 / wpb;
    b = std::min(b, (int)((160 * 1024) / (lds > 0 ? lds : 1)));
    b = std::min(b, 32 / wpb);
    return std::max(1, b);
}

size_t mvhdp_sweep_wave_bytes(int M, int S_cap);
size_t mvhdp_sweep_fast_wave_bytes(int M, int S_cap, int rmax);

struct PlanTuning {
    int force_primary = 0;
    int narrow = -1;
    int walk_fixed = 0;
    double walk_theta[MVHDP_MAXM] = {0};
    double primary_min_share = 0.10;
    int single_stream = 0;
    int four_round_on_c = -1;
    int delta16 = 1;
    int narrow_wide = 1;
    int fork_delay_us = 0;
    int widest_on_main = 0;
    int live_overlap = -1;
    int single_wave = 0;
    int live16 = -1;
    int live_rows = -1;
    int live_rows_segments = 1;
    int coef_lds_max_bytes = 12 * 1024;
    double live_rows_theta = 0.3;
};

enum { WALK_GROUPS = 3 };
struct WalkTuner {
    int walk_i = 0, walk_probe_i = 0, walk_b_i = 0, walk_phase = 0, walk_dir = 1, walk_fails = 0, walk_wait = 4, walk_cfg = -1, walk_maxj = 6;
    bool walk_far = false;
    double walk_ns_a1 = 0.0, walk_ns_b = 0.0;
    int walk_cls = 2, walk_i_by[WALK_GROUPS] = {-1, -1, -1};
    int walk_default[WALK_GROUPS] = {0, 0, 0};

    void init_defaults(int K)
    {
        if (K >= 256) { walk_default[0] = 6; walk_default[1] = MVHDP_WALK_BINS; walk_default[2] = 9; }
        walk_i = walk_default[walk_cls];
    }
    int stored(int g) const { return walk_i_by[g] >= 0 ? walk_i_by[g] : walk_default[g]; }
    double walk_cap = 0.004;
    long long walk_idle_until = 0, walk_refresh_at = 0, sweeps_done = 0;
    double walk_f[MVHDP_MAXM] = {-1, -1, -1, -1, -1, -1, -1, -1};
    double walk_hist[MVHDP_WALK_BINS] = {0};

    bool controlled(int m) const { return walk_f[m] >= 0.0 && walk_f[m] < 0.35; }
    bool any_controlled(int M) const { for (int m = 0; m < M; m++) if (controlled(m)) return true; return false; }
    bool any_unknown(int M) const { for (int m = 0; m < M; m++) if (walk_f[m] < 0.0) return true; return false; }

    void propose(int grp, int M, double theta[WALK_GROUPS][MVHDP_MAXM], bool* measure)
    {
        if (grp != walk_cls) {
            walk_i_by[walk_cls] = walk_i;
            walk_i = stored(grp);
            walk_cls = grp;
            walk_phase = 0; walk_far = false;
        }
        const bool any = any_controlled(M);
        const int top = MVHDP_WALK_BINS;
        walk_probe_i = walk_i;
        if (walk_phase == 1 && any) {
            if (walk_far && walk_i < 4) walk_far = false;
            if (walk_far) walk_dir = -1;
            if (walk_dir > 0 && walk_i >= top) walk_dir = -1;
            if (walk_dir < 0 && walk_i <= 0) walk_dir = 1;
            if (walk_dir > 0) {
                int j = 1;
                double extra = walk_hist[walk_i];
                while (walk_i + j < top && j < walk_maxj && extra + walk_hist[walk_i + j] <= walk_cap) { extra += walk_hist[walk_i + j]; j++; }
                walk_probe_i = walk_i + j;
            } else walk_probe_i = walk_far ? walk_i / 2 : walk_i - 1;
        }
        for (int m = 0; m < MVHDP_MAXM; m++) {
            const bool c = m < M && controlled(m);
            for (int g = 0; g < WALK_GROUPS; g++) theta[g][m] = c ? (double)(g == grp ? walk_probe_i : stored(g)) / MVHDP_WALK_BINS : 0.0;
        }
        *measure = false;
        if (!any && sweeps_done >= walk_refresh_at) { *measure = true; walk_refresh_at = sweeps_done + 16; }
        if (any_unknown(M)) *measure = true;
    }

    void measured(int M, int nseg, const unsigned long long* view_stats )
    {
        double all = 0.0;
        for (int m = 0; m < M; m++) {
            const double n = (double)view_stats[m * MVHDP_VIEW_STATS];
            all += n;
            if (n >= 64) walk_f[m] = (double)view_stats[m * MVHDP_VIEW_STATS + 1] / n;
            else if (nseg == 1) walk_f[m] = 1.0;
        }
        for (int b = 0; b < MVHDP_WALK_BINS; b++) {
            double c = 0.0;
            for (int m = 0; m < M; m++)
                if (controlled(m)) c += (double)view_stats[m * MVHDP_VIEW_STATS + 2 + b];
            walk_hist[b] = all > 0 ? c / all : 0.0;
        }
    }

    void observe(bool comparable, int cfg, int M, double ns)
    {
        sweeps_done++;
        const bool any = any_controlled(M);
        if (!comparable || walk_cfg != cfg) {
            walk_phase = 0;
            walk_cfg = comparable ? cfg : -1;
            if (comparable) walk_ns_a1 = 0.0;
// ... 134 lines not shown
    auto geometry = [&](bool is_fast, int c, int walk, ClassLaunch& g) -> bool {
        const int r = 1 << c;
        g.fast = is_fast; g.r = is_fast ? r : 0;
        g.S_cap = is_fast ? std::min(S_cap, 64 * r) : S_cap;
        g.wave_bytes = (uint32_t)(is_fast ? mvhdp_sweep_fast_wave_bytes(M, g.S_cap, r) : mvhdp_sweep_wave_bytes(M, S_cap));
        g.wpb = 4;
        while (g.wpb > 1 && p.block_shared_bytes + (size_t)g.wpb * g.wave_bytes > in.max_lds) g.wpb >>= 1;
        g.lds = p.block_shared_bytes + (size_t)g.wpb * g.wave_bytes;
        if (g.lds > in.max_lds) return false;
        const int regs = is_fast ? in.regs.regs[c][in.debug ? 2 : (walk ? 1 : 0)] : in.regs.regs[5][in.debug ? 2 : 0];
        const int bpc = plan_blocks_per_cu(regs, 64 * g.wpb, g.lds);
        const int64_t need = (in.D + (int64_t)g.wpb * MVHDP_DOC_BATCH - 1) / ((int64_t)g.wpb * MVHDP_DOC_BATCH);
        g.grid = (int)std::max<int64_t>(1, std::min<int64_t>(need, (int64_t)in.num_cus * ((p.overlap && bpc > 1) ? bpc - 1 : bpc)));
        if (tu.single_wave) { g.wpb = 1; g.lds = p.block_shared_bytes + g.wave_bytes; g.grid = 1; }
        return true;
    };

    const bool mirror_ok = fast && !in.debug && tu.narrow != 0 && (!(flags & MVHDP_SWEEP_REUSE_TREES) || in.trees_current) &&
                           !((flags & MVHDP_SWEEP_SEGMENT_OVERLAP) && in.unassigned);
    const bool want_live16 = mirror_ok && p.live && !p.frozen && !in.unassigned && (tu.live16 > 0 || (tu.live16 < 0 && K >= 256));
    auto group_of = [&](int c) { return c != 0 ? 2 : ((mirror_ok && (!p.live || want_live16)) ? 0 : 1); };
    double theta[WALK_GROUPS][MVHDP_MAXM] = {{0}};
    bool measure = false;
    if (tu.walk_fixed) {
        for (int g = 0; g < WALK_GROUPS; g++) for (int m = 0; m < MVHDP_MAXM; m++) theta[g][m] = tu.walk_theta[m];
        measure = true;
    } else wt.propose(fast ? group_of(p.dominant) : 2, M, theta, &measure);
    const bool mirror_pays = mirror_ok && !p.live && K >= 256;
    auto walk_of = [&](int c) { const int g = group_of(c); bool w = measure || in.debug || mirror_pays; for (int m = 0; m < M; m++) w = w || theta[g][m] > 0.0; return w ? 1 : 0; };

    ClassLaunch gen;
    if (!geometry(false, 5, 0, gen)) return fail(MVHDP_ERR_UNSUPPORTED, "per-entity LDS state exceeds 160 KiB (K * modalities too large)");
    gen.used = false;
    if (fast) {
        ClassLaunch pg;
        if (!geometry(true, pc, walk_of(pc), pg)) fast = false;
    }
    p.fast = fast;
    p.pc = fast ? pc : 5;
    const bool four_on_c = tu.four_round_on_c > 0 || (tu.four_round_on_c < 0 && !unknown && tok[2] < 0.03 * tot);
    const int stream_of[MVHDP_N_CLASSES] = {PLAN_STREAM_C, PLAN_STREAM_C, four_on_c ? PLAN_STREAM_C : PLAN_STREAM_D, PLAN_STREAM_B, PLAN_STREAM_A, PLAN_STREAM_A};
    if (!fast) {
        p.cls[5] = gen; p.cls[5].used = true; p.cls[5].stream = PLAN_STREAM_MAIN;
        for (int c = 0; c < MVHDP_N_CLASSES; c++) p.class_map[c] = 5;
        p.route = false; p.H = 0;
        p.need_full = true;
    } else {
        p.H = (S_cap > (64 << pc)) ? (in.have_order ? in.n_longer[pc] : in.D) : 0;
        if (view_16 && pc >= 3) p.H = in.have_order ? std::max<int64_t>(p.H, in.n_longer[4]) : in.D;
        p.route = p.H > 0;
        for (int c = pc; c < MVHDP_N_CLASSES; c++) {
            const bool reachable = c == pc || (p.route && (c <= c_max || (c == 5 && view_16)));
            const bool populated = c == pc || unknown || in.ent_hist[c] != 0 || (c == 5 && view_16);
            if (!(reachable && populated)) continue;
            ClassLaunch g;
            const int w = walk_of(c);
            if (c < 5 && geometry(true, c, w, g)) { g.walk = w; }
            else { g = gen; g.walk = 0; }
            g.used = true;
            g.stream = (c == pc || tu.single_stream || tu.single_wave) ? PLAN_STREAM_MAIN : stream_of[c];
            for (int m = 0; m < MVHDP_MAXM; m++) g.theta[m] = theta[group_of(c)][m];
            p.cls[c] = g;
        }
        if (!tu.single_stream && !tu.single_wave && tu.widest_on_main) {
            int next = PLAN_STREAM_MAIN;
            for (int c = MVHDP_N_CLASSES - 1; c >= pc; c--) if (p.cls[c].used) { p.cls[c].stream = next; next = std::min(next + 1, (int)PLAN_STREAM_D); }
        }
        for (int c = 0; c < MVHDP_N_CLASSES; c++) {
            int t = std::max(c, pc);
            while (t < MVHDP_N_CLASSES && !p.cls[t].used) t++;
            p.class_map[c] = t < MVHDP_N_CLASSES ? t : -1;
        }
        p.need_full = in.debug;
        for (int c = pc; c < MVHDP_N_CLASSES; c++) if (p.cls[c].used && !p.cls[c].fast) p.need_full = true;
        if (p.route && p.class_map[5] < 0 && (c_max == 5 || view_16)) {
            p.cls[5] = gen; p.cls[5].used = true; p.cls[5].stream = tu.single_stream ? PLAN_STREAM_MAIN : PLAN_STREAM_A; p.class_map[5] = 5; p.need_full = true;
        }
    }
    if (mirror_ok && !p.live && p.cls[0].used && p.cls[0].fast && p.cls[0].walk) p.cls[0].narrow = 1;
    if (mirror_ok && !p.live && tu.narrow_wide && tu.narrow != 1)
        for (int c = 1; c < 5; c++) if (p.cls[c].used && p.cls[c].fast && p.cls[c].walk) p.cls[c].narrow = 1;
    p.delta16 = tu.delta16 != 0 && mirror_ok && !p.live && !p.frozen && !p.seg_apply && nseg == 1 && p.only_seg < 0 &&
                !(flags & MVHDP_SWEEP_NO_APPLY) && !in.unassigned;
    if (want_live16) {
        bool all_fast = true;
        for (int c = 0; c < MVHDP_N_CLASSES; c++) if (p.cls[c].used && !p.cls[c].fast) all_fast = false;
        if (all_fast) {
            p.live16 = true;
            for (int c = 0; c < MVHDP_N_CLASSES; c++) if (p.cls[c].used) { p.cls[c].walk = 1; p.cls[c].narrow = 1; }
        }
    }
    if (want_rows) {
        bool all_fast = p.fast;
        for (int c = 0; c < MVHDP_N_CLASSES; c++) if (p.cls[c].used && !p.cls[c].fast) all_fast = false;
        if (all_fast) {
            p.live_rows = true;
            p.need_full = false;
            for (int c = 0; c < MVHDP_N_CLASSES; c++)
                if (p.cls[c].used) {
                    p.cls[c].walk = 1;
                    for (int m = 0; m < MVHDP_MAXM; m++) p.cls[c].theta[m] = (m < M && wt.controlled(m)) ? tu.live_rows_theta : 0.0;
                }
        } else p.coef_lds = false;
    } else p.coef_lds = false;
    p.walk_cfg = (p.live_rows ? 1 << 20 : 0) + (p.fast ? (1 << p.dominant) : 32) * 2 + (p.route ? 1 : 0) + 64 * nseg + (p.live ? 1 << 16 : 0) + (p.seg_apply ? 1 << 17 : 0) + (p.live16 ? 1 << 18 : 0) + (p.overlap ? 1 << 19 : 0);
}
```

### mvtopicmodel_amd/csrc/mvhdp_sweep_fast.hip

```cpp
#include "mvhdp_device.h"
#include "../../include/mvhdp.h"
#include "mvhdp_wave.h"

size_t mvhdp_sweep_fast_wave_bytes(int M, int S_cap, int rmax)
{
    size_t counts = (size_t)M * S_cap * (rmax >= 8 ? 2 : 4);
    size_t b = (size_t)(64 + 64 + 64 + 16 + S_cap) * 4 + counts;
    b += (size_t)M * M * 12;
    return (b + 15) & ~(size_t)15;
}

#ifndef MVHDP_LB1
#define MVHDP_LB1 1
#endif
#ifndef MVHDP_LB1W
#define MVHDP_LB1W 7
#endif
#ifndef MVHDP_LB2
#define MVHDP_LB2 7
#endif
#ifndef MVHDP_LB2_ROOMY
#define MVHDP_LB2_ROOMY 6
#endif
#ifndef MVHDP_LB4
#define MVHDP_LB4 4
#endif
#ifndef MVHDP_NB2_FROM
#define MVHDP_NB2_FROM 4
#endif
#ifndef MVHDP_LB16
#define MVHDP_LB16 1
#endif
#ifndef MVHDP_LB_ROWS
#define MVHDP_LB_ROWS 7
#endif
#ifndef MVHDP_LB8
#define MVHDP_LB8 1
#endif
#ifndef MVHDP_GATHER_SC
#define MVHDP_GATHER_SC 0
#endif
template <typename T>
__device__ __forceinline__ int gather_cell(gptr_t p)
{
    const __attribute__((address_space(1))) T* q = (const __attribute__((address_space(1))) T*)p;
#if MVHDP_GATHER_SC == 1
    return (int)__hip_atomic_load(q, __ATOMIC_RELAXED, __HIP_MEMORY_SCOPE_AGENT);
#elif MVHDP_GATHER_SC == 3
    return (int)__hip_atomic_load(q, __ATOMIC_RELAXED, __HIP_MEMORY_SCOPE_SYSTEM);
#elif MVHDP_GATHER_SC == 4
    return (int)__builtin_nontemporal_load(q);
#else
    return (int)*q;
#endif
}
#define W_HEAVY 0x40000000
#define W_BIG   0x20000000
#define W_ROW(w) ((w) & 0x1fffffff)
typedef unsigned int rowq_t __attribute__((ext_vector_type(4), aligned(4)));
typedef float coefq_t __attribute__((ext_vector_type(4)));

__device__ __forceinline__ int smoothing_sample_live(const float* __restrict__ smp, int K, float t, int lane)
{
    for (int k0 = 0; k0 < K; k0 += WAVE) {
        const int k = k0 + lane;
        const float p = (k < K) ? smp[k] : 3.0e38f;
        const unsigned long long hit = __builtin_amdgcn_ballot_w64(p > t && k < K);
        if (hit) return k0 + (int)__builtin_ctzll(hit);
    }
    return K - 1;
}

template <bool CELL16>
__device__ __forceinline__ rowq_t row_batch_load(gptr_t rowp, int K, int b, int lane)
{
    constexpr int CPL = CELL16 ? 8 : 4;
    const int k = (b * WAVE + lane) * CPL;
    rowq_t q = {0u, 0u, 0u, 0u};
    if (k < K) q = *(const __attribute__((address_space(1))) rowq_t*)(rowp + (unsigned int)k * (CELL16 ? 2u : 4u));
    return q;
}

typedef float f2_t __attribute__((ext_vector_type(2)));
template <bool CELL16>
__device__ __forceinline__ int row_batch_pick(rowq_t q, coefq_t c0, coefq_t c1, int kb, float base, float target, bool force, float& tot, bool& any)
{
    constexpr int CPL = CELL16 ? 8 : 4, NS = CPL / 2;
    f2_t n2[NS], k2[NS], A[NS];
    if (CELL16) {
        n2[0] = f2_t{(float)(q.x & 0xffffu), (float)(q.x >> 16)}; n2[1] = f2_t{(float)(q.y & 0xffffu), (float)(q.y >> 16)};
        n2[NS - 2] = f2_t{(float)(q.z & 0xffffu), (float)(q.z >> 16)}; n2[NS - 1] = f2_t{(float)(q.w & 0xffffu), (float)(q.w >> 16)};
        k2[0] = f2_t{c0.x, c0.y}; k2[1] = f2_t{c0.z, c0.w}; k2[NS - 2] = f2_t{c1.x, c1.y}; k2[NS - 1] = f2_t{c1.z, c1.w};
    } else {
        n2[0] = f2_t{(float)(int)q.x, (float)(int)q.y}; n2[NS - 1] = f2_t{(float)(int)q.z, (float)(int)q.w};
        k2[0] = f2_t{c0.x, c0.y}; k2[NS - 1] = f2_t{c0.z, c0.w};
    }
    A[0] = n2[0] * k2[0];
#pragma unroll
    for (int s = 1; s < NS; s++) A[s] = __builtin_elementwise_fma(n2[s], k2[s], A[s - 1]);
    const float ev = A[NS - 1].x;
    const float acc = ev + A[NS - 1].y;
    const float incl = wave_incl_scan_f_dpp(acc);
    tot = bcast_f(incl, 63);
    const unsigned long long pos = __builtin_amdgcn_ballot_w64(acc > 0.0f);
    any = pos != 0;
    if (!pos || !(force || base + tot > target)) return -1;
    const unsigned long long hit = force ? 0ull : (__builtin_amdgcn_ballot_w64(base + incl > target) & pos);
    const int hl = hit ? (int)__builtin_ctzll(hit) : 63 - (int)__builtin_clzll(pos);
    const float thr = target - (base + (hl > 0 ? bcast_f(incl, hl - 1) : 0.0f));
    int cnt = 0;
#pragma unroll
    for (int s = 0; s < NS; s++) cnt += (A[s].x <= thr) ? 1 : 0;
#pragma unroll
    for (int s = 0; s < NS; s++) cnt += (ev + A[s].y <= thr) ? 1 : 0;
    int p = force ? CPL : bcast_i(cnt, hl);
    if (p >= CPL) {
        int lp = 0;
#pragma unroll
        for (int s = 0; s < NS; s++) if (n2[s].x > 0.0f && k2[s].x > 0.0f) lp = s;
#pragma unroll
        for (int s = 0; s < NS; s++) if (n2[s].y > 0.0f && k2[s].y > 0.0f) lp = NS + s;
        p = bcast_i(lp, hl);
    }
    return kb + hl * CPL + (p < NS ? 2 * p : 2 * (p - NS) + 1);
}

template <bool CELL16, bool TWOB>
__device__ __forceinline__ int row_sample_live(rowq_t q0, bool have_q0, bool in_lds, const __attribute__((address_space(3))) float* cf_lds, const float* __restrict__ cf_g, const float* __restrict__ smp, float S,
                                                gptr_t rowp, int K, float u2f, float rootf, int bq, float mass0, int lane, unsigned long long* t_after_wait)
{
    constexpr int CPL = CELL16 ? 8 : 4;
    (void)t_after_wait;
    float target = u2f * rootf;
    if (target < S) return smoothing_sample_live(smp, K, target, lane);
    target -= S;
    float base = 0.0f;
    int lastb = -1;
    const int nb = (K + WAVE * CPL - 1) / (WAVE * CPL);
    if (!TWOB || nb != 2) bq = 0;
    const float bbase = bq ? mass0 : 0.0f;
    if (have_q0 && in_lds) {
// ... 226 lines not shown
            const double pmj = pd ? pd[lane] : 1.0;
            qsh[lane] = pmj * (mm.gamma[pj] * mm.alpha[(int64_t)pj * (K + 1) + K]) / dd;
            wsh[lane] = (pj != pm && wlen[pj] != 0) ? (float)(pmj / dd) : 0.0f;
        }
        LDS_FENCE();
        MVHDP_TMAIN(tp, tt, te);
        bool aborted = false;

        for (int m = 0; m < M && !aborted; m++) {
            const int lenm = uniform_i(wlen[m]);
            if (lenm == 0) continue;
            const double beta_m = mm.beta[m];
            const double scale_m = (double)lenm + mm.gamma[m] * mm.alpha_sum[m];
            const double p_mm = pd ? pd[m * M + m] : 1.0;
            const int32_t* nk = nk_all + (int64_t)m * K;

            int cn[RMAX];
            double oth[RMAX], den[RMAX];
            unsigned int onz = 0;
            auto slot_consts = [&](int r, double& o, double& dn) {
                o = 0.0; dn = 1.0;
                const int i = lane * R_eff + r;
                if (r < R_eff && i < S_used) {
                    const int k = koff[r] >> 2;
                    double acc = 0.0;
                    for (int j = 0; j < M; j++) {
                        if (j == m) continue;
                        const int cj = sn_get(j * S + i);
                        const int lj = wlen[j];
                        if (lj != 0)
                            acc += pd[m * M + j] * ((double)cj + mm.gamma[j] * mm.alpha[(int64_t)j * (K + 1) + k])
                                   / ((double)lj + mm.gamma[j] * mm.alpha_sum[j]);
                    }
                    o = acc * scale_m;
                    dn = (double)nk[k] + mm.beta_sum[m];
                }
            };
            float rden32[RMAX], brden32[RMAX], oth32[RMAX];
            const float beta32 = (float)beta_m, scale32 = (float)scale_m;
            const float* const smp_m = mm.coef + (int64_t)M * Kp + (int64_t)m * K;
            const float smS = LIVEROWS ? uniform_f(smp_m[K - 1]) : 0.0f;
#pragma unroll
            for (int r = 0; r < RMAX; r++) {
                cn[r] = 0;
                const int i = lane * R_eff + r;
                const bool used = r < R_eff && i < S_used;
                if (SCREEN) {
                    float acc = 0.0f;
                    double dn = 1.0;
                    if (used) {
                        const int k = koff[r] >> 2;
                        cn[r] = sn_get(m * S + i);
                        for (int j = 0; j < M; j++) {
                            if (j == m) continue;
                            const int cj = sn_get(j * S + i);
                            if (cj != 0) onz |= 1u << r;
                            acc = __builtin_fmaf(wsh[m * M + j], (float)cj + (float)(mm.gamma[j] * mm.alpha[(int64_t)j * (K + 1) + k]), acc);
                        }
                        dn = (double)nk[k] + mm.beta_sum[m];
                    }
                    oth[r] = 0.0; den[r] = 1.0;
                    rden32[r] = __builtin_amdgcn_rcpf((float)dn);
                    brden32[r] = beta32 * rden32[r];
                    oth32[r] = acc * scale32;
                } else {
                    if (used) {
                        cn[r] = sn_get(m * S + i);
                        for (int j = 0; j < M; j++) if (j != m && sn_get(j * S + i) != 0) onz |= 1u << r;
                    }
                    slot_consts(r, oth[r], den[r]);
                    rden32[r] = 0.0f; brden32[r] = 0.0f; oth32[r] = 0.0f;
                }
            }
            double newAll = 0.0;
            for (int j = 0; j < M; j++) newAll += qsh[m * M + j];
            newAll = newAll * scale_m;
            const double newMass = (mm.first_inactive < 0) ? 0.0 : newAll / (double)K;
            const float pmm32 = uniform_f((float)p_mm), newMass32 = uniform_f((float)newMass);

            const int64_t base = mm.doc_off[m][d];
            const int64_t row0 = mm.rowbase[m];
            const char* nwk_v = (const char*)(nwk + row0 * K);
            const char* nwk16_v = (const char*)(nwk16 + row0 * K);
            int koffh[RMAX];
#pragma unroll
            for (int r = 0; r < RMAX; r++) koffh[r] = koff[r] >> 1;
            const int Vm = mm.V[m];
            const double walk_theta = sl.walk_theta[m];
            const unsigned int v_tok0 = n_tok, v_tree0 = c_tree;
            unsigned int whist_l = 0;

            MVHDP_TMAIN(tv, te, te);
            for (int c0 = 0; c0 < lenm && !aborted; c0 += WAVE) {
                const int ti = c0 + lane;
                const bool tvalid = ti < lenm;
                int w_l = tvalid ? mm.tok[m][base + ti] : -1;
                int z_l = tvalid ? mm.z[m][base + ti] : -1;
                int so_l = -1;
                if (z_l >= 0) {
                    uint32_t w = bitmap[z_l >> 5];
                    so_l = prefix[z_l >> 5] + __popc(w & ((1u << (z_l & 31)) - 1u));
                }
                double u1_l, u2_l;
                {
                    uint32_t x[4];
                    philox4x32_10((uint32_t)ti, (uint32_t)m, (uint32_t)dg, sl.sweep_idx,
                                  sl.seed_lo, sl.seed_hi ^ (uint32_t)((unsigned long long)dg >> 32), x);
                    u1_l = bits_to_unit(x[0], x[1]);
                    u2_l = bits_to_unit(x[2], x[3]);
                }
                MVHDP_TSUB2(tp);
                if (w_l >= Vm) w_l = -1;
                if (NARROW && w_l >= 0) {
                    const int hv = mm.heavy[row0 + w_l];
                    if (hv) w_l |= (hv == MVHDP_ROW_HEAVY) ? (W_HEAVY | W_BIG) : W_BIG;
                }
                const float u1f_l = (float)u1_l;
                int znew_l = z_l;

                double root_l = 0.0;
                int zt_l = -1, st_l = -1;
                const bool heavy_l = NARROW && w_l >= 0 && (w_l & W_HEAVY);
                const bool walk_l = tvalid && w_l >= 0 && (!WALK || u1_l >= walk_theta) && (!LIVEROWS || heavy_l);
                const unsigned long long walked = WALK ? __ballot(walk_l) : ~0ull;
                const unsigned long long specm = LIVEROWS ? __ballot(tvalid && w_l >= 0 && !heavy_l && u1_l >= walk_theta) : 0ull;
                rowq_t rowq = {0u, 0u, 0u, 0u};
                if (WALK && tvalid && w_l >= 0 && !walk_l) root_l = mm.root[row0 + W_ROW(w_l)];
                {
                    const bool act = walk_l;
                    const double* __restrict__ dt = mm.dtab + (row0 + W_ROW(max(w_l, 0))) * (int64_t)mm.dt_nblk * 8;
                    double u = 0.0;
                    int i = 1;
                    for (int bd = 0; bd < mm.dt_nbd; bd++) {
                        if (act && (bd == 0 || i < K)) {
                            const double2* __restrict__ blk = (const double2*)(dt + (int64_t)(mm.dt_base[bd] + (i - (1 << mm.dt_depth[bd]))) * 8);
                            double2 q0, q1, q2, q3;
                            if (LIVEROWS) {
                                const double* bp = (const double*)blk;
                                q0.x = __hip_atomic_load(bp + 0, __ATOMIC_RELAXED, __HIP_MEMORY_SCOPE_AGENT); q0.y = __hip_atomic_load(bp + 1, __ATOMIC_RELAXED, __HIP_MEMORY_SCOPE_AGENT);
                                q1.x = __hip_atomic_load(bp + 2, __ATOMIC_RELAXED, __HIP_MEMORY_SCOPE_AGENT); q1.y = __hip_atomic_load(bp + 3, __ATOMIC_RELAXED, __HIP_MEMORY_SCOPE_AGENT);
                                q2.x = __hip_atomic_load(bp + 4, __ATOMIC_RELAXED, __HIP_MEMORY_SCOPE_AGENT); q2.y = __hip_atomic_load(bp + 5, __ATOMIC_RELAXED, __HIP_MEMORY_SCOPE_AGENT);
                                q3.x = __hip_atomic_load(bp + 6, __ATOMIC_RELAXED, __HIP_MEMORY_SCOPE_AGENT); q3.y = __hip_atomic_load(bp + 7, __ATOMIC_RELAXED, __HIP_MEMORY_SCOPE_AGENT);
                            } else { q0 = blk[0]; q1 = blk[1]; q2 = blk[2]; q3 = blk[3]; }
                            const int levels = (bd == 0) ? mm.dt_f : 3;
                            if (bd == 0) { root_l = q3.y; u = u2_l * root_l; }
                            int path = 0;
                            if (i < K && levels > 0) {
                                const double l = q0.x;
                                if (u < l) { i = 2 * i; } else { u = u - l; i = 2 * i + 1; path = 1; }
                            }
                            if (i < K && levels > 1) {
                                const double l = path ? q1.x : q0.y;
                                if (u < l) { i = 2 * i; path = 2 * path; } else { u = u - l; i = 2 * i + 1; path = 2 * path + 1; }
                                if (i < K && levels > 2) {
                                    const double l3 = (path == 0) ? q1.y : (path == 1) ? q2.x : (path == 2) ? q2.y : q3.x;
                                    if (u < l3) { i = 2 * i; } else { u = u - l3; i = 2 * i + 1; }
                                }
                            }
                        }
                    }
                    if (act) {
                        zt_l = i - K;
                        const uint32_t wbit = bitmap[zt_l >> 5];
                        if ((wbit >> (zt_l & 31)) & 1u) st_l = (int)(prefix[zt_l >> 5] + __popc(wbit & ((1u << (zt_l & 31)) - 1u)));
                    }
                }

                MVHDP_TSUB2(tv);
                const float root32_l = (float)root_l;
                const float u2f_l = LIVEROWS ? (float)u2_l : 0.0f;
                unsigned long long bselm = 0ull;
                if (LIVEROWS == 2) {
                    constexpr int BCELLS = WAVE * (NARROW ? 8 : 4);
                    if (K > BCELLS && K <= 2 * BCELLS) {
                        float mass0_l = 0.0f;
                        if (tvalid && w_l >= 0 && !heavy_l) mass0_l = mm.mass0[row0 + W_ROW(w_l)];
                        bselm = __ballot(tvalid && w_l >= 0 && !heavy_l && (u2f_l * root32_l) - smS >= mass0_l);
                    }
                }
                MVHDP_TMAIN(th, te, tt);
                constexpr int NB = (RMAX >= MVHDP_NB2_FROM) ? 2 : 1;
                int gn[RMAX], gn2[RMAX];
                unsigned long long rem = __ballot(tvalid && w_l >= 0);
                n_oov += (unsigned int)__popcll(__ballot(tvalid && w_l < 0));
                n_tok += (unsigned int)__popcll(rem);
                const int t_first = rem ? (int)__builtin_ctzll(rem) : 0;
#pragma unroll
                for (int a = 0; a < NB; a++) {
                    const unsigned long long ra = (a == 0) ? rem : (rem & (rem - 1));
                    const int w0 = bcast_i(w_l, ra ? (int)__builtin_ctzll(ra) : t_first);
                    const unsigned int r0 = (unsigned int)W_ROW(max(w0, 0));
                    const bool h0 = w0 >= 0 && (w0 & W_HEAVY);
                    if (NARROW && !h0) {
                        const gptr_t c0q = scalar_row(nwk16_v, r0, (unsigned int)K * 2u);
#pragma unroll
                        for (int r = 0; r < RMAX; r++) { const int v = gather_cell<uint16_t>(c0q + (unsigned int)koffh[r]); if (a == 0) gn[r] = v; else gn2[r] = v; }
                    } else {
                        const gptr_t c0p = scalar_row(nwk_v, r0, (unsigned int)K * 4u);
#pragma unroll
                        for (int r = 0; r < RMAX; r++) { const int v = gather_cell<int32_t>(c0p + (unsigned int)koff[r]); if (a == 0) gn[r] = v; else gn2[r] = v; }
                    }
                }

                while (rem) {
                    const int t = (int)__builtin_ctzll(rem);
                    rem &= ~(1ull << t);
#define TOK_T t
#define TOK_G gn
#include "mvhdp_sweep_fast_token.inc"
#undef TOK_T
#undef TOK_G
                    if (NB == 2 && rem) {
                        const int t1 = (int)__builtin_ctzll(rem);
                        rem &= ~(1ull << t1);
#define TOK_T t1
#define TOK_G gn2
#include "mvhdp_sweep_fast_token.inc"
#undef TOK_T
#undef TOK_G
                    }
                }

                MVHDP_TMAIN(tt, te, te);
                {
                    const bool chg = tvalid && (w_l >= 0) && (znew_l != z_l) && !(sl.flags & MVHDP_SWEEP_FROZEN);
                    n_chg += (unsigned int)__popcll(__ballot(chg));
                    if (chg) {
                        const int64_t rowK = (row0 + W_ROW(w_l)) * K;
                        if (NARROW && sl.live16 && !(w_l & W_HEAVY)) {
                            unsigned int* m32 = (unsigned int*)mm.counts16;
                            if (z_l >= 0) { const int64_t c = rowK + z_l; __hip_atomic_fetch_add(&m32[c >> 1], 0u - (1u << ((c & 1) * 16)), __ATOMIC_RELAXED, __HIP_MEMORY_SCOPE_AGENT); }
                            { const int64_t c = rowK + znew_l; __hip_atomic_fetch_add(&m32[c >> 1], 1u << ((c & 1) * 16), __ATOMIC_RELAXED, __HIP_MEMORY_SCOPE_AGENT); }
                        } else if (NARROW && sl.delta16 && !(w_l & W_BIG)) {
                            unsigned int* d32 = (unsigned int*)mm.delta16;
                            if (z_l >= 0) { const int64_t c = rowK + z_l; __hip_atomic_fetch_add(&d32[c >> 1], 0u - (1u << ((c & 1) * 16)), __ATOMIC_RELAXED, __HIP_MEMORY_SCOPE_AGENT); }
                            { const int64_t c = rowK + znew_l; __hip_atomic_fetch_add(&d32[c >> 1], 1u << ((c & 1) * 16), __ATOMIC_RELAXED, __HIP_MEMORY_SCOPE_AGENT); }
                        } else {
#ifdef MVHDP_PROBE
                            const int probe = (int)((sl.flags >> 16) & 7u);
                            int64_t c_old = rowK + z_l, c_new = rowK + znew_l;
                            if (probe == 1) { c_old &= 0xffff; c_new &= 0xffff; }
                            if (probe == 7) { c_old &= 0xfffff; c_new &= 0xfffff; }
                            if (probe == 5) { c_old &= 0x7fffff; c_new &= 0x7fffff; }
                            if (probe == 6) { c_old &= 0xffffff; c_new &= 0xffffff; }
                            if (probe == 3) { if (z_l >= 0) dnwk[c_old] = -1; dnwk[c_new] = 1; }
                            else if (probe == 4) { if (z_l >= 0) __hip_atomic_fetch_add(&dnwk[c_old], -1, __ATOMIC_RELAXED, __HIP_MEMORY_SCOPE_WORKGROUP); __hip_atomic_fetch_add(&dnwk[c_new], 1, __ATOMIC_RELAXED, __HIP_MEMORY_SCOPE_WORKGROUP); }
                            else {
                                if (z_l >= 0) __hip_atomic_fetch_add(&dnwk[c_old], -1, __ATOMIC_RELAXED, __HIP_MEMORY_SCOPE_AGENT);
                                if (probe != 2) __hip_atomic_fetch_add(&dnwk[c_new], 1, __ATOMIC_RELAXED, __HIP_MEMORY_SCOPE_AGENT);
                            }
#else
                            if (z_l >= 0) __hip_atomic_fetch_add(&dnwk[rowK + z_l], -1, __ATOMIC_RELAXED, __HIP_MEMORY_SCOPE_AGENT);
                            __hip_atomic_fetch_add(&dnwk[rowK + znew_l], 1, __ATOMIC_RELAXED, __HIP_MEMORY_SCOPE_AGENT);
#endif
                        }
                        if (z_l >= 0) {
                            if (sl.nk_global) __hip_atomic_fetch_add(&dnk_g[m * K + z_l], -1, __ATOMIC_RELAXED, __HIP_MEMORY_SCOPE_AGENT);
                            else __hip_atomic_fetch_add(&nkd[m * K + z_l], -1, __ATOMIC_RELAXED, __HIP_MEMORY_SCOPE_WORKGROUP);
                        }
                        if (sl.nk_global) __hip_atomic_fetch_add(&dnk_g[m * K + znew_l], 1, __ATOMIC_RELAXED, __HIP_MEMORY_SCOPE_AGENT);
                        else __hip_atomic_fetch_add(&nkd[m * K + znew_l], 1, __ATOMIC_RELAXED, __HIP_MEMORY_SCOPE_WORKGROUP);
                        if (mm.first_inactive >= 0 && mm.inactive[znew_l]) {
                            long long key = (long long)MVHDP_ACT_KEY(dg, m, ti, znew_l);
                            atomicMin(sl.act_key, key);
                            if (sl.births) {
                                const int r_ = sl.births[2 + K + znew_l];
                                if (r_ >= 0) { atomicMin(&sl.birth_keys[r_], key); atomicMax(&sl.births[0], r_ + 1); }
                            }
                        }
                    }
                }
                if (tvalid) mm.z[m][base + ti] = znew_l;
                if (tvalid && znew_l >= 0) atomicOr(&bitmap2[znew_l >> 5], 1u << (znew_l & 31));
                if (sl.flags & MVHDP_SL_STRICT_LIVE) {
                    asm volatile("s_waitcnt vmcnt(0)" ::: "memory");
                    __builtin_amdgcn_fence(__ATOMIC_ACQUIRE, "agent");
                }
                MVHDP_TMAIN(te, te, te);
            }

#pragma unroll
            for (int r = 0; r < RMAX; r++) {
                const int i = lane * R_eff + r;
                if (r < R_eff && i < S_used) sn_set(m * S + i, cn[r]);
            }
            if (WALK && n_tok != v_tok0) {
                const unsigned int v = lane < MVHDP_WALK_BINS ? whist_l : lane == MVHDP_WALK_BINS ? n_tok - v_tok0 : c_tree - v_tree0;
                const int idx = lane < MVHDP_WALK_BINS ? 2 + lane : lane - MVHDP_WALK_BINS;
                if (lane < MVHDP_WALK_BINS + 2 && v) atomicAdd(&vstat_s[m * MVHDP_VIEW_STATS + idx], v);
            }
            LDS_FENCE();
        }
        if (aborted) n_abort++;
        LDS_FENCE();
        {
            int c2 = __popc(lane < NW ? bitmap2[lane] : 0u);
#pragma unroll
            for (int sft = 32; sft >= 1; sft >>= 1) c2 += __shfl_xor(c2, sft, WAVE);
            if (lane == 0) {
                mm.nslots[d] = aborted ? (uint16_t)MVHDP_NSLOTS_UNKNOWN : (uint16_t)c2;
                if (sl.slot_hist) {
                    if (c2 > 0) atomicAdd(&hist_s[min((c2 + 63) >> 6, MVHDP_HIST_BINS) - 1], (unsigned int)doc_tokens);
// ... 162 lines not shown
```

### mvtopicmodel_amd/csrc/mvhdp_sweep_fast_token.inc

```
{
                    int g[RMAX];
#pragma unroll
                    for (int r = 0; r < RMAX; r++) g[r] = TOK_G[r];
                    const int wfull_t = LIVEROWS ? bcast_i(w_l, TOK_T) : 0;
                    const gptr_t rowp_t = !LIVEROWS ? (gptr_t)0 : NARROW ? scalar_row(nwk16_v, (unsigned int)W_ROW(wfull_t), (unsigned int)K * 2u)
                                                                         : scalar_row(nwk_v, (unsigned int)W_ROW(wfull_t), (unsigned int)K * 4u);
                    const bool spec_t = LIVEROWS && ((specm >> TOK_T) & 1ull);
                    const int bsel_t = (LIVEROWS == 2) ? (int)((bselm >> TOK_T) & 1ull) : 0;
                    if (LIVEROWS) {
#pragma unroll
                        for (int r = 0; r < RMAX; r++) asm volatile("" : "+v"(g[r]));
                        if (spec_t) rowq = row_batch_load<NARROW>(rowp_t, K, bsel_t, lane);
                    }
                    const unsigned long long rem_n = (NB == 2) ? (rem & (rem - 1)) : rem;
#pragma unroll
                    for (int r = 0; r < RMAX; r++) { touch_lane_off(koff[r]); if (NARROW) touch_lane_off(koffh[r]); }
                    if (NB == 2 || LIVEROWS || rem_n) {
                        const int wn = bcast_i(w_l, rem_n ? (int)__builtin_ctzll(rem_n) : TOK_T);
                        if (NARROW && !(wn & W_HEAVY)) {
                            const gptr_t cnq = scalar_row(nwk16_v, (unsigned int)W_ROW(wn), (unsigned int)K * 2u);
#pragma unroll
                            for (int r = 0; r < RMAX; r++) TOK_G[r] = gather_cell<uint16_t>(cnq + (unsigned int)koffh[r]);
                        } else {
                            const gptr_t cnp = scalar_row(nwk_v, (unsigned int)W_ROW(wn), (unsigned int)K * 4u);
#pragma unroll
                            for (int r = 0; r < RMAX; r++) TOK_G[r] = gather_cell<int32_t>(cnp + (unsigned int)koff[r]);
                        }
                    }
                    const int w = W_ROW(bcast_i(w_l, TOK_T));
                    const int so = bcast_i(so_l, TOK_T);
                    const int64_t row = row0 + w;

                    if (so >= 0) {
                        const int rs = so & (R_eff - 1), ls = so >> lg;
#pragma unroll
                        for (int r = 0; r < RMAX; r++) {
                            if (rs == r) {
                                const int c = bcast_i(cn[r], ls) - 1;
                                cn[r] = wave_writelane(cn[r], c, ls);
                                if (c == 0 && !((bcast_i((int)onz, ls) >> r) & 1)) live_m[r] &= ~(1ull << ls);
                            }
                        }
                    }

                    double mass = 0.0, s0 = 0.0, s1 = 0.0, total = 0.0;
                    int branch = 2, slot_new = -1;
                    bool unsafe = false;
                    double term[RMAX] = {};
                    bool need64 = DEBUG || exact_only || !SCREEN;
                    if (SCREEN && !need64) {
                        const float u1f = bcast_f(u1f_l, TOK_T), rootf = bcast_f(root32_l, TOK_T);
                        float t32[RMAX], c32v[RMAX];
#pragma unroll
                        for (int r = 0; r < RMAX; r++) {
                            const float pw = __builtin_fmaf((float)g[r], rden32[r], brden32[r]);
                            const float a32 = __builtin_fmaf(pmm32, (float)cn[r], oth32[r]);
                            t32[r] = __builtin_amdgcn_inverse_ballot_w64(live_m[r]) ? a32 * pw : 0.0f;
                        }
                        float ls = t32[0];
                        c32v[0] = ls;
#pragma unroll
                        for (int r = 1; r < RMAX; r++) { ls += t32[r]; c32v[r] = ls; }
                        const float incl = wave_incl_scan_f_dpp(ls);
                        const float excl = incl - ls;
#pragma unroll
                        for (int r = 0; r < RMAX; r++) c32v[r] = (r == RMAX - 1) ? incl : excl + c32v[r];
                        const float massf = bcast_f(incl, 63);
                        const float totalf = (newMass32 + massf) + rootf;
                        const float s0f = u1f * totalf;
                        const float tolf = totalf * 0x1.0p-17f;
                        bool close;
                        if (s0f < newMass32) {
                            branch = 0;
                            close = fabsf(s0f - newMass32) <= tolf;
                        } else {
                            const float s1f = s0f - newMass32;
                            close = (fabsf(s1f) <= tolf) || (fabsf(s1f - massf) <= tolf);
                            if (s1f < massf) {
                                branch = 1;
                                unsigned long long anyhit = 0, near = 0, hitr[RMAX];
#pragma unroll
                                for (int r = 0; r < RMAX; r++) {
                                    const float diff = c32v[r] - s1f;
                                    near |= __builtin_amdgcn_ballot_w64(fabsf(diff) <= tolf) & live_m[r];
                                    hitr[r] = __builtin_amdgcn_ballot_w64(diff >= 0.0f) & live_m[r];
                                    anyhit |= hitr[r];
                                }
                                close = close || near != 0;
                                if (anyhit) {
                                    if (RMAX <= 4) {
                                        unsigned int best = ~0u;
#pragma unroll
                                        for (int r = 0; r < RMAX; r++) {
                                            const unsigned int fl = hitr[r] ? (unsigned int)__builtin_ctzll(hitr[r]) : 0x0fffffffu;
                                            best = min(best, fl * (unsigned int)R_eff + (unsigned int)r);
                                        }
                                        slot_new = (int)best;
                                    } else {
                                        const int hl = (int)__builtin_ctzll(anyhit);
                                        int rr = 0;
#pragma unroll
                                        for (int r = RMAX - 1; r >= 0; r--) if ((hitr[r] >> hl) & 1ull) rr = r;
                                        slot_new = hl * R_eff + rr;
                                    }
                                } else close = true;
                            } else {
// ... 191 lines not shown
```

Measured before the change: 6.770 billion.

## Add 8-bit word-topic count mirror with exception tail for narrow gathers

Adds a per-row uint8 mirror of word-topic counts. Rows with at most four cells of 255 or more store those overflow values in a small tail that one scalar vector load reads. The tree-build kernel fills this mirror and marks such rows with a byte class bit. The narrow sweep path then gathers byte cells instead of 16-bit cells, patching capped values from the tail. The goal is to halve gather bandwidth and cache footprint, at the cost of extra build work, a ballot-guarded patch loop per token, and a smaller vocabulary limit.

```diff
diff --git a/include/mvhdp.h b/include/mvhdp.h
--- a/include/mvhdp.h
+++ b/include/mvhdp.h
@@ -201,6 +201,7 @@
     double  tree_branch_share[MVHDP_MAX_MODALITIES];
     int32_t live_overlap;
     int32_t live_rows;
+    int32_t byte8;
 } mvhdp_tuning;
 int mvhdp_get_tuning(mvhdp_handle h, mvhdp_tuning* t);
 int mvhdp_set_tuning(mvhdp_handle h, const mvhdp_tuning* t);
diff --git a/mvtopicmodel_amd/_lib.py b/mvtopicmodel_amd/_lib.py
--- a/mvtopicmodel_amd/_lib.py
+++ b/mvtopicmodel_amd/_lib.py
@@ -69,7 +69,7 @@
                 ("live16", C.c_int32), ("single_wave", C.c_int32),
                 ("walk_theta", C.c_double * MAX_M), ("primary_min_share", C.c_double),
                 ("learnt_walk_step", C.c_int32 * 4), ("tree_branch_share", C.c_double * MAX_M),
-                ("live_overlap", C.c_int32), ("live_rows", C.c_int32)]
+                ("live_overlap", C.c_int32), ("live_rows", C.c_int32), ("byte8", C.c_int32)]
 
 
 class GroupInfoC(C.Structure):
diff --git a/mvtopicmodel_amd/csrc/mvhdp_api.hip b/mvtopicmodel_amd/csrc/mvhdp_api.hip
--- a/mvtopicmodel_amd/csrc/mvhdp_api.hip
+++ b/mvtopicmodel_amd/csrc/mvhdp_api.hip
@@ -46,6 +46,7 @@
     if (const char* f = getenv("MVHDP_GATE_PCT")) { const int v = atoi(f); if (v >= 5 && v <= 95) h->gate_pct = v; }
     if (const char* f = getenv("MVHDP_FOUR_ROUND_ON_C")) h->tu.four_round_on_c = atoi(f);
     if (const char* f = getenv("MVHDP_DELTA16")) h->tu.delta16 = atoi(f) != 0;
+    if (const char* f = getenv("MVHDP_BYTE8")) h->tu.byte8 = atoi(f) != 0 ? -1 : 0;
     if (const char* f = getenv("MVHDP_FORK_DELAY_US")) h->tu.fork_delay_us = std::max(0, std::min(1000, atoi(f)));
     if (const char* f = getenv("MVHDP_FORCE_MODE")) { if (!strcmp(f, "serial")) h->tu.single_stream = 1; }
     if (const char* f = getenv("MVHDP_PRIMARY_MIN_SHARE")) { const double v = atof(f); if (v > 0.0 && v <= 1.0) h->tu.primary_min_share = v; }
@@ -76,7 +77,7 @@
         return MVHDP_ERR_INVALID_ARG;
     }
     for (int m = 0; m < M; m++) if (cfg->num_types[m] < 1) { g_create_error = "num_types[m] must be >= 1"; return MVHDP_ERR_INVALID_ARG; }
-    for (int m = 0; m < M; m++) if (cfg->num_types[m] >= (1 << 29)) { g_create_error = "num_types[m] must be below 2^29"; return MVHDP_ERR_INVALID_ARG; }
+    for (int m = 0; m < M; m++) if (cfg->num_types[m] >= (1 << 28)) { g_create_error = "num_types[m] must be below 2^28"; return MVHDP_ERR_INVALID_ARG; }
     if (cfg->doc_id_base < 0 || cfg->doc_id_base >= (1LL << 29)) { g_create_error = "doc_id_base out of range"; return MVHDP_ERR_INVALID_ARG; }
     int ndev = 0;
     if (hipGetDeviceCount(&ndev) != hipSuccess || ndev <= 0 || cfg->device < 0 || cfg->device >= ndev) {
@@ -117,6 +118,8 @@
     CREATE_HIP(hipMemset(mm.counts16, 0, (size_t)nrows * K * sizeof(uint16_t)));
     CREATE_HIP(hipMalloc(&mm.delta16, (size_t)(nrows * K + 2) * sizeof(uint16_t)));
     CREATE_HIP(hipMemsetD16(mm.delta16, (unsigned short)0x8000, (size_t)(nrows * K + 2)));
+    CREATE_HIP(hipMalloc(&mm.counts8, (size_t)nrows * c8_stride(K)));
+    CREATE_HIP(hipMemset(mm.counts8, 0, (size_t)nrows * c8_stride(K)));
     CREATE_HIP(hipMalloc(&mm.heavy, (size_t)nrows));
     CREATE_HIP(hipMemset(mm.heavy, 1, (size_t)nrows));
     CREATE_HIP(hipMemset(mm.delta, 0, cbytes));
@@ -175,7 +178,7 @@
     if (h->stream) hipStreamSynchronize(h->stream);
     auto fr = [](auto*& p) { if (p) { hipFree((void*)p); p = nullptr; } };
     for (int m = 0; m < MVHDP_MAXM; m++) { fr(h->d_doc_off[m]); fr(h->d_tok[m]); fr(h->d_z[m]); fr(h->d_carry[m]); fr(h->d_present[m]); }
-    fr(h->mm.counts); fr(h->mm.delta16); fr(h->mm.counts16); fr(h->mm.heavy); fr(h->mm.delta); fr(h->mm.trees); fr(h->mm.root); fr(h->mm.coef); fr(h->mm.mass0); fr(h->d_births); fr(h->d_birth_keys); fr(h->d_birth_table); fr(h->mm.dtab); fr(h->mm.p);
+    fr(h->mm.counts); fr(h->mm.delta16); fr(h->mm.counts16); fr(h->mm.counts8); fr(h->mm.heavy); fr(h->mm.delta); fr(h->mm.trees); fr(h->mm.root); fr(h->mm.coef); fr(h->mm.mass0); fr(h->d_births); fr(h->d_birth_keys); fr(h->d_birth_table); fr(h->mm.dtab); fr(h->mm.p);
     fr(h->d_alpha); fr(h->d_inactive); fr(h->d_ctl);
     if (h->h_ctl) { hipHostFree(h->h_ctl); h->h_ctl = nullptr; }
     h->d_stats = nullptr; h->d_act_key = nullptr; h->d_doc_counter = nullptr; h->d_ovf_meta = nullptr;
@@ -1088,6 +1091,7 @@
     sl.live_rows = p.live_rows ? 1 : 0;
     sl.coef_lds = p.coef_lds ? 1 : 0;
     sl.delta16 = p.delta16 ? 1 : 0;
+    sl.byte8 = p.byte8 ? 1 : 0;
     sl.stats = d_stats;
     sl.act_key = h->d_act_key;
     const bool births = sweep_births(p, flags, mm);
@@ -1514,7 +1518,7 @@
     memset(t, 0, sizeof *t);
     t->force_primary = h->tu.force_primary; t->narrow = h->tu.narrow; t->walk_fixed = h->tu.walk_fixed;
     t->single_stream = h->tu.single_stream; t->primary_min_share = h->tu.primary_min_share; t->live16 = h->tu.live16;
-    t->single_wave = h->tu.single_wave; t->live_overlap = h->tu.live_overlap; t->live_rows = h->tu.live_rows;
+    t->single_wave = h->tu.single_wave; t->live_overlap = h->tu.live_overlap; t->live_rows = h->tu.live_rows; t->byte8 = h->tu.byte8;
     for (int m = 0; m < MVHDP_MAX_MODALITIES; m++) { t->walk_theta[m] = h->tu.walk_theta[m]; t->tree_branch_share[m] = h->wt.walk_f[m]; }
     for (int g = 0; g < WALK_GROUPS; g++) t->learnt_walk_step[g] = g == h->wt.walk_cls ? h->wt.walk_i : h->wt.walk_i_by[g];
     t->learnt_walk_step[3] = -1;
@@ -1535,6 +1539,7 @@
     h->tu.single_wave = t->single_wave ? 1 : 0;
     h->tu.live_overlap = t->live_overlap < 0 ? -1 : (t->live_overlap ? 1 : 0);
     h->tu.live_rows = t->live_rows < 0 ? -1 : (t->live_rows ? 1 : 0);
+    h->tu.byte8 = t->byte8 < 0 ? -1 : (t->byte8 ? 1 : 0);
     h->tu.primary_min_share = t->primary_min_share > 0.0 ? t->primary_min_share : 0.10;
     for (int m = 0; m < MVHDP_MAX_MODALITIES; m++) h->tu.walk_theta[m] = t->walk_theta[m];
     if (t->learnt_walk_step[0] >= 0 || t->learnt_walk_step[1] >= 0 || t->learnt_walk_step[2] >= 0) h->wt.restore(t->learnt_walk_step, t->tree_branch_share, h->mm.M);
@@ -1560,7 +1565,7 @@
     wt.init_defaults(in.K);
     if (t) {
         tu.force_primary = t->force_primary; tu.narrow = t->narrow; tu.walk_fixed = t->walk_fixed; tu.single_stream = t->single_stream;
-        tu.live16 = t->live16; tu.single_wave = t->single_wave ? 1 : 0; tu.live_overlap = t->live_overlap; tu.live_rows = t->live_rows;
+        tu.live16 = t->live16; tu.single_wave = t->single_wave ? 1 : 0; tu.live_overlap = t->live_overlap; tu.live_rows = t->live_rows; tu.byte8 = t->byte8;
         if (t->primary_min_share > 0) tu.primary_min_share = t->primary_min_share;
         for (int m = 0; m < MVHDP_MAX_MODALITIES; m++) tu.walk_theta[m] = t->walk_theta[m];
         if (t->learnt_walk_step[0] >= 0 || t->learnt_walk_step[1] >= 0 || t->learnt_walk_step[2] >= 0) wt.restore(t->learnt_walk_step, t->tree_branch_share, in.M);
diff --git a/mvtopicmodel_amd/csrc/mvhdp_device.h b/mvtopicmodel_amd/csrc/mvhdp_device.h
--- a/mvtopicmodel_amd/csrc/mvhdp_device.h
+++ b/mvtopicmodel_amd/csrc/mvhdp_device.h
@@ -20,6 +20,7 @@
     int32_t* counts;
     uint16_t* delta16;
     uint16_t* counts16;
+    uint8_t* counts8;
     uint8_t* heavy;
     int32_t* delta;
     double* trees;
@@ -40,6 +41,11 @@
 #define MVHDP_SL_STRICT_LIVE 0x8000u
 #define MVHDP_ROW_HEAVY 1
 #define MVHDP_ROW_BIG 2
+#define MVHDP_ROW_BYTE 4
+#define MVHDP_ROW_CLASS(h) ((h) & 3)
+#define MVHDP_C8_E 4
+__host__ __device__ inline int c8_tail(int K) { return (K + 3) & ~3; }
+__host__ __device__ inline int c8_stride(int K) { return (c8_tail(K) + 4 * MVHDP_C8_E + 15) & ~15; }
 
 struct SweepLaunch {
     uint32_t sweep_idx;
@@ -62,6 +68,7 @@
     double walk_theta[MVHDP_MAXM];
     int32_t walk;
     int32_t narrow;
+    int32_t byte8;
     int32_t delta16;
     int32_t live16;
     int32_t live_rows;
diff --git a/mvtopicmodel_amd/csrc/mvhdp_group.hip b/mvtopicmodel_amd/csrc/mvhdp_group.hip
--- a/mvtopicmodel_amd/csrc/mvhdp_group.hip
+++ b/mvtopicmodel_amd/csrc/mvhdp_group.hip
@@ -469,6 +469,7 @@
     std::vector<uint8_t> cls((size_t)rows);
     GHIP(g, hipSetDevice(L0->device));
     GHIP(g, hipMemcpy(cls.data(), L0->mm.heavy, (size_t)rows, hipMemcpyDeviceToHost));
+    for (uint8_t& c : cls) c = (uint8_t)MVHDP_ROW_CLASS(c);
     g->woff.assign((size_t)rows + 1, 0);
     for (int64_t r = 0; r < rows; r++) g->woff[(size_t)r + 1] = g->woff[(size_t)r] + (cls[(size_t)r] == 0 ? (K + 1) / 2 : K);
     if (g->d_woff.empty()) { g->d_woff.assign(g->leaders.size(), nullptr); g->d_cls.assign(g->leaders.size(), nullptr); g->xpack.assign(g->leaders.size(), nullptr); }
diff --git a/mvtopicmodel_amd/csrc/mvhdp_kernels.hip b/mvtopicmodel_amd/csrc/mvhdp_kernels.hip
--- a/mvtopicmodel_amd/csrc/mvhdp_kernels.hip
+++ b/mvtopicmodel_amd/csrc/mvhdp_kernels.hip
@@ -107,8 +107,11 @@
         const double* al = mm.alpha + (int64_t)m * (K + 1);
         const double beta = mm.beta[m], beta_sum = mm.beta_sum[m], gamma = mm.gamma[m];
         uint16_t* c16 = mm.counts16 + row * K;
-        const bool light_src = from_mirror && mm.heavy[row] != MVHDP_ROW_HEAVY;
+        uint8_t* c8 = mm.counts8 + row * c8_stride(K);
+        const int cls_in = mm.heavy[row];
+        const bool light_src = from_mirror && cls_in != MVHDP_ROW_HEAVY;
         bool hv = false;
+        int cls = MVHDP_ROW_CLASS(cls_in);
         if (!from_mirror) {
             long long sum = 0;
             for (int k0 = 0; k0 < K; k0 += WAVE * TB) {
@@ -135,8 +138,10 @@
 #pragma unroll
             for (int sft = 32; sft >= 1; sft >>= 1) sum += __shfl_xor(sum, sft, WAVE);
             hv = sum > 65534;
-            if (lane == 0) mm.heavy[row] = hv ? MVHDP_ROW_HEAVY : (sum > 32767 ? MVHDP_ROW_BIG : 0);
-        }
+            cls = hv ? MVHDP_ROW_HEAVY : (sum > 32767 ? MVHDP_ROW_BIG : 0);
+        }
+        unsigned int tw = 0xFFFFFFFFu;
+        int nlarge = 0;
         for (int k0 = 0; k0 < K; k0 += WAVE * TB) {
             int cv[TB], nkv[TB];
             double alv[TB];
@@ -157,6 +162,7 @@
                     const int c = cv[u];
                     if (light_src) cnt[k] = c;
                     else if (!from_mirror) c16[k] = hv ? (uint16_t)65535 : (uint16_t)c;
+                    c8[k] = (uint8_t)min(max(c, 0), 255);
                     double leaf;
                     if (inference_leaves) {
                         leaf = ((double)c + beta) / ((double)nkv[u] + beta_sum);
@@ -169,7 +175,23 @@
                     t[K + k] = leaf;
                 }
             }
-        }
+#pragma unroll
+            for (int u = 0; u < TB; u++) {
+                const int k = k0 + u * WAVE + lane;
+                unsigned long long big = __ballot(k < K && cv[u] >= 255);
+                while (big && nlarge < MVHDP_C8_E) {
+                    const int src = (int)__builtin_ctzll(big);
+                    const unsigned int w = (unsigned int)__shfl(((k0 + u * WAVE + lane) << 16) | ((cv[u] - 255) & 0xffff), src, WAVE);
+                    if (lane == nlarge) tw = w;
+                    nlarge++;
+                    big &= big - 1;
+                }
+                nlarge += __popcll(big);
+            }
+        }
+        if (lane < MVHDP_C8_E) *(unsigned int*)(c8 + c8_tail(K) + 4 * lane) = tw;
+        const int cls_out = cls | ((cls != MVHDP_ROW_HEAVY && nlarge <= MVHDP_C8_E) ? MVHDP_ROW_BYTE : 0);
+        if (lane == 0 && cls_out != cls_in) mm.heavy[row] = (uint8_t)cls_out;
         tree_from_leaves(mm, row, t, lane, write_full);
     }
     if (apply_first && negatives) {
diff --git a/mvtopicmodel_amd/csrc/mvhdp_plan.h b/mvtopicmodel_amd/csrc/mvhdp_plan.h
--- a/mvtopicmodel_amd/csrc/mvhdp_plan.h
+++ b/mvtopicmodel_amd/csrc/mvhdp_plan.h
@@ -63,6 +63,7 @@
     bool need_full = false;
     int nk_global = 0;
     uint32_t block_shared_bytes = 0;
+    bool byte8 = false;
     bool delta16 = false;
     bool live16 = false;
     bool live_rows = false;
@@ -117,6 +118,7 @@
     int live_rows = -1;
     int live_rows_segments = 1;
     int coef_lds_max_bytes = 12 * 1024;
+    int byte8 = -1;
     double live_rows_theta = 0.3;
 };
 
@@ -417,6 +419,7 @@
         for (int c = 1; c < 5; c++) if (p.cls[c].used && p.cls[c].fast && p.cls[c].walk) p.cls[c].narrow = 1;
     p.delta16 = tu.delta16 != 0 && mirror_ok && !p.live && !p.frozen && !p.seg_apply && nseg == 1 && p.only_seg < 0 &&
                 !(flags & MVHDP_SWEEP_NO_APPLY) && !in.unassigned;
+    p.byte8 = tu.byte8 != 0 && mirror_ok && !p.live && !p.overlap && !(flags & MVHDP_SWEEP_REUSE_TREES);
     if (want_live16) {
         bool all_fast = true;
         for (int c = 0; c < MVHDP_N_CLASSES; c++) if (p.cls[c].used && !p.cls[c].fast) all_fast = false;
diff --git a/mvtopicmodel_amd/csrc/mvhdp_sweep_fast.hip b/mvtopicmodel_amd/csrc/mvhdp_sweep_fast.hip
--- a/mvtopicmodel_amd/csrc/mvhdp_sweep_fast.hip
+++ b/mvtopicmodel_amd/csrc/mvhdp_sweep_fast.hip
@@ -56,7 +56,14 @@
 }
 #define W_HEAVY 0x40000000
 #define W_BIG   0x20000000
-#define W_ROW(w) ((w) & 0x1fffffff)
+#define W_BYTE  0x10000000
+#define W_ROW(w) ((w) & 0x0fffffff)
+typedef unsigned int c8tail_t __attribute__((ext_vector_type(4), aligned(4)));
+static_assert(MVHDP_C8_E == 4, "one s_load_dwordx4 per tail");
+__device__ __forceinline__ c8tail_t load_c8_tail(gptr_t row, int tail_off)
+{
+    return *(const __attribute__((address_space(4))) c8tail_t*)(uintptr_t)(row + tail_off);
+}
 typedef unsigned int rowq_t __attribute__((ext_vector_type(4), aligned(4)));
 typedef float coefq_t __attribute__((ext_vector_type(4)));
 
@@ -449,6 +456,8 @@
             const int64_t row0 = mm.rowbase[m];
             const char* nwk_v = (const char*)(nwk + row0 * K);
             const char* nwk16_v = (const char*)(nwk16 + row0 * K);
+            const int c8s = c8_stride(K), c8t = c8_tail(K);
+            const char* nwk8_v = (const char*)(mm.counts8 + row0 * c8s);
             int koffh[RMAX];
 #pragma unroll
             for (int r = 0; r < RMAX; r++) koffh[r] = koff[r] >> 1;
@@ -480,7 +489,8 @@
                 if (w_l >= Vm) w_l = -1;
                 if (NARROW && w_l >= 0) {
                     const int hv = mm.heavy[row0 + w_l];
-                    if (hv) w_l |= (hv == MVHDP_ROW_HEAVY) ? (W_HEAVY | W_BIG) : W_BIG;
+                    if (MVHDP_ROW_CLASS(hv)) w_l |= (MVHDP_ROW_CLASS(hv) == MVHDP_ROW_HEAVY) ? (W_HEAVY | W_BIG) : W_BIG;
+                    if (sl.byte8 && (hv & MVHDP_ROW_BYTE)) w_l |= W_BYTE;
                 }
                 const float u1f_l = (float)u1_l;
                 int znew_l = z_l;
@@ -548,6 +558,8 @@
                 MVHDP_TMAIN(th, te, tt);
                 constexpr int NB = (RMAX >= MVHDP_NB2_FROM) ? 2 : 1;
                 int gn[RMAX], gn2[RMAX];
+                constexpr bool BYTE8 = NARROW && !LIVEROWS;
+                c8tail_t tl = {~0u, ~0u, ~0u, ~0u}, tl2 = tl;
                 unsigned long long rem = __ballot(tvalid && w_l >= 0);
                 n_oov += (unsigned int)__popcll(__ballot(tvalid && w_l < 0));
                 n_tok += (unsigned int)__popcll(rem);
@@ -558,7 +570,12 @@
                     const int w0 = bcast_i(w_l, ra ? (int)__builtin_ctzll(ra) : t_first);
                     const unsigned int r0 = (unsigned int)W_ROW(max(w0, 0));
                     const bool h0 = w0 >= 0 && (w0 & W_HEAVY);
-                    if (NARROW && !h0) {
+                    if (BYTE8 && w0 >= 0 && (w0 & W_BYTE)) {
+                        const gptr_t c0b = scalar_row(nwk8_v, r0, (unsigned int)c8s);
+                        if (a == 0) tl = load_c8_tail(c0b, c8t); else tl2 = load_c8_tail(c0b, c8t);
+#pragma unroll
+                        for (int r = 0; r < RMAX; r++) { const int v = gather_cell<uint8_t>(c0b + (unsigned int)(koffh[r] >> 1)); if (a == 0) gn[r] = v; else gn2[r] = v; }
+                    } else if (NARROW && !h0) {
                         const gptr_t c0q = scalar_row(nwk16_v, r0, (unsigned int)K * 2u);
 #pragma unroll
                         for (int r = 0; r < RMAX; r++) { const int v = gather_cell<uint16_t>(c0q + (unsigned int)koffh[r]); if (a == 0) gn[r] = v; else gn2[r] = v; }
@@ -574,17 +591,21 @@
                     rem &= ~(1ull << t);
 #define TOK_T t
 #define TOK_G gn
+#define TOK_TL tl
 #include "mvhdp_sweep_fast_token.inc"
 #undef TOK_T
 #undef TOK_G
+#undef TOK_TL
                     if (NB == 2 && rem) {
                         const int t1 = (int)__builtin_ctzll(rem);
                         rem &= ~(1ull << t1);
 #define TOK_T t1
 #define TOK_G gn2
+#define TOK_TL tl2
 #include "mvhdp_sweep_fast_token.inc"
 #undef TOK_T
 #undef TOK_G
+#undef TOK_TL
                     }
                 }
 
diff --git a/mvtopicmodel_amd/csrc/mvhdp_sweep_fast_token.inc b/mvtopicmodel_amd/csrc/mvhdp_sweep_fast_token.inc
--- a/mvtopicmodel_amd/csrc/mvhdp_sweep_fast_token.inc
+++ b/mvtopicmodel_amd/csrc/mvhdp_sweep_fast_token.inc
@@ -2,6 +2,21 @@
                     int g[RMAX];
 #pragma unroll
                     for (int r = 0; r < RMAX; r++) g[r] = TOK_G[r];
+                    if (BYTE8 && TOK_TL[0] != ~0u) {
+                        bool capped = false;
+#pragma unroll
+                        for (int r = 0; r < RMAX; r++) capped = capped || g[r] == 255;
+                        if (__ballot(capped)) {
+#pragma unroll
+                            for (int e = 0; e < MVHDP_C8_E; e++) {
+                                const unsigned int tw = TOK_TL[e];
+                                if (tw == ~0u) break;
+                                const int th = (int)(tw >> 16) * 2, tv = 255 + (int)(tw & 0xffffu);
+#pragma unroll
+                                for (int r = 0; r < RMAX; r++) g[r] = (koffh[r] == th) ? tv : g[r];
+                            }
+                        }
+                    }
                     const int wfull_t = LIVEROWS ? bcast_i(w_l, TOK_T) : 0;
                     const gptr_t rowp_t = !LIVEROWS ? (gptr_t)0 : NARROW ? scalar_row(nwk16_v, (unsigned int)W_ROW(wfull_t), (unsigned int)K * 2u)
                                                                          : scalar_row(nwk_v, (unsigned int)W_ROW(wfull_t), (unsigned int)K * 4u);
@@ -17,11 +32,18 @@
                     for (int r = 0; r < RMAX; r++) { touch_lane_off(koff[r]); if (NARROW) touch_lane_off(koffh[r]); }
                     if (NB == 2 || LIVEROWS || rem_n) {
                         const int wn = bcast_i(w_l, rem_n ? (int)__builtin_ctzll(rem_n) : TOK_T);
-                        if (NARROW && !(wn & W_HEAVY)) {
+                        if (BYTE8 && (wn & W_BYTE)) {
+                            const gptr_t cnb = scalar_row(nwk8_v, (unsigned int)W_ROW(wn), (unsigned int)c8s);
+                            TOK_TL = load_c8_tail(cnb, c8t);
+#pragma unroll
+                            for (int r = 0; r < RMAX; r++) TOK_G[r] = gather_cell<uint8_t>(cnb + (unsigned int)(koffh[r] >> 1));
+                        } else if (NARROW && !(wn & W_HEAVY)) {
                             const gptr_t cnq = scalar_row(nwk16_v, (unsigned int)W_ROW(wn), (unsigned int)K * 2u);
+                            if (BYTE8) TOK_TL = c8tail_t{~0u, ~0u, ~0u, ~0u};
 #pragma unroll
                             for (int r = 0; r < RMAX; r++) TOK_G[r] = gather_cell<uint16_t>(cnq + (unsigned int)koffh[r]);
                         } else {
+                            if (BYTE8) TOK_TL = c8tail_t{~0u, ~0u, ~0u, ~0u};
                             const gptr_t cnp = scalar_row(nwk_v, (unsigned int)W_ROW(wn), (unsigned int)K * 4u);
 #pragma unroll
                             for (int r = 0; r < RMAX; r++) TOK_G[r] = gather_cell<int32_t>(cnp + (unsigned int)koff[r]);
```

After: 6.749 billion (median of 6 runs). No clear change (-0.3%).
